# google-research/weatherbenchX

Hardware: AMD Instinct MI355X
Metric: grid-point·metric evals/s (0.25° 721×1440×37L) at 1/2/4/8 GPUs; % HBM roofline (higher is better)
Workload: dtype f32+f64

## Files before the change

include/wbx.h:

```cpp
#ifndef WBX_H_
#define WBX_H_

#include <stddef.h>
#include <stdint.h>

#ifdef __cplusplus
extern "C" {
#endif

#define WBX_ABI_VERSION 13

typedef enum wbx_status {
  WBX_OK = 0,
  WBX_ERR_INVALID = -1,
  WBX_ERR_HIP = -2,
  WBX_ERR_NO_DEVICE = -3,
  WBX_ERR_FFT = -4,
  WBX_ERR_RCCL = -5
} wbx_status;

typedef struct wbx_ctx wbx_ctx;

typedef enum wbx_dtype { WBX_F32 = 0, WBX_F64 = 1 } wbx_dtype;

typedef enum wbx_det_func { WBX_DET3 = 0, WBX_DET6 = 1, WBX_PASS1 = 2 } wbx_det_func;
#define WBX_DET3_LANES 3
#define WBX_DET6_LANES 6
#define WBX_PASS1_LANES 1

#define WBX_ENS_LANES 5
typedef enum wbx_ens_algo {
  WBX_ENS_SORT = 0,
  WBX_ENS_PAIRWISE = 1
} wbx_ens_algo;

#define WBX_FLAG_MASKED 1u
#define WBX_FLAG_SKIPNA 2u
#define WBX_FLAG_FAIR   4u
#define WBX_FLAG_SKIPNA_ENS 8u

#define WBX_MAX_INPUTS 4

typedef struct wbx_s1_plan {
  int64_t nkey;
  int64_t ndepth;
  int64_t nx;
  int32_t x_kept;
  int32_t nchunk;
  int64_t depth_chunk;
  int64_t xstride[WBX_MAX_INPUTS];
  const int64_t* key_off[WBX_MAX_INPUTS];
  const int64_t* depth_off[WBX_MAX_INPUTS];
  const int32_t* gather_key;
  const int32_t* gather_depth;
  const int64_t* gather_tab;
  int32_t n_gather_depth;
  uint32_t flags;
  int32_t block_threads;
  int32_t vec;
  int32_t plane_rows;
  int32_t reserved_;
  const double* x_weights;
} wbx_s1_plan;

int wbx_s1_partial_len(const wbx_s1_plan* plan, int lanes, int64_t* n_out);

int wbx_abi_version(void);
const char* wbx_last_error(void);
int wbx_device_count(int* n_out);
int wbx_ctx_create(int device_id, void* hip_stream, wbx_ctx** out);
int wbx_ctx_destroy(wbx_ctx* ctx);
int wbx_ctx_synchronize(wbx_ctx* ctx);
int wbx_ctx_device_name(wbx_ctx* ctx, char* buf, size_t buflen);

int wbx_malloc(wbx_ctx* ctx, size_t bytes, void** dptr_out);
int wbx_free(wbx_ctx* ctx, void* dptr);
int wbx_memcpy_h2d(wbx_ctx* ctx, void* dptr, const void* h_src, size_t bytes);
int wbx_memcpy_d2h(wbx_ctx* ctx, void* h_dst, const void* dptr, size_t bytes);
int wbx_memset(wbx_ctx* ctx, void* dptr, int value, size_t bytes);

typedef struct wbx_fence wbx_fence;
int wbx_host_alloc(wbx_ctx* ctx, size_t bytes, void** h_out);
int wbx_host_free(wbx_ctx* ctx, void* h_ptr);
int wbx_memcpy_d2h_async(wbx_ctx* ctx, void* h_pinned, const void* dptr, size_t bytes);
int wbx_fence_create(wbx_ctx* ctx, wbx_fence** out);
int wbx_fence_record(wbx_ctx* ctx, wbx_fence* fence);
int wbx_fence_wait(wbx_fence* fence);
int wbx_fence_destroy(wbx_fence* fence);
int wbx_ctx_wait_fence(wbx_ctx* ctx, wbx_fence* fence);
int wbx_memcpy_h2d_async(wbx_ctx* ctx, void* dptr, const void* h_pinned, size_t bytes);
int wbx_memcpy_d2d(wbx_ctx* ctx, void* dst, const void* src, size_t bytes);
int wbx_host_transpose(void* dst, const void* src, int64_t batch, int64_t rows, int64_t cols, int32_t elem_bytes);
int wbx_clock_probe(wbx_ctx* ctx, int32_t blocks, double* shader_mhz_out);

int wbx_acc_add(wbx_ctx* ctx, double* acc, const double* src, int64_t n, int32_t overwrite);

#define WBX_COMM_ID_BYTES 128
typedef struct wbx_comm wbx_comm;
int wbx_comm_unique_id(void* id_out );
int wbx_comm_create(wbx_ctx* ctx, const void* unique_id, int32_t nranks, int32_t rank, wbx_comm** out);
int wbx_comm_destroy(wbx_comm* comm);
int wbx_comm_info(const wbx_comm* comm, int32_t* nranks_out, int32_t* rank_out, int64_t* collectives_out);
int wbx_acc_allreduce(wbx_ctx* ctx, wbx_comm* comm, double* acc, int64_t n);
int wbx_acc_read(wbx_ctx* ctx, const double* acc, int64_t n, double* host_out);
int wbx_acc_reset(wbx_ctx* ctx, double* acc, int64_t n);

int wbx_notnan_mask(wbx_ctx* ctx, const void* data, int dtype, int64_t n, uint8_t* valid_out);

int wbx_timer_start(wbx_ctx* ctx);
int wbx_timer_stop(wbx_ctx* ctx, float* ms_out);
int wbx_mark(wbx_ctx* ctx, int* index_out);
int wbx_mark_elapsed(wbx_ctx* ctx, int i0, int i1, float* ms_out);
int wbx_marks_reset(wbx_ctx* ctx);

int wbx_det_partial(wbx_ctx* ctx, const wbx_s1_plan* plan, int func ,
                    int dtype , const void* p, const void* t, const void* c,
                    const uint8_t* mask, double* partial_out);

int wbx_ens_partial(wbx_ctx* ctx, const wbx_s1_plan* plan, int dtype, int M,
                    int64_t member_stride, int algo , const void* p,
                    const void* t, const uint8_t* mask, double* partial_out);

#define WBX_ENS2_LANES 2
int wbx_ens2_partial(wbx_ctx* ctx, const wbx_s1_plan* plan, int dtype, int M, int64_t member_stride, int N,
                     int64_t target_member_stride, const void* p, const void* t, const uint8_t* mask, double* partial_out);

typedef struct wbx_s2_plan {
  int64_t nA, nBk, nBr, nchunk, nlane, nj, nbin;
  int32_t sum_j;
} wbx_s2_plan;
int wbx_contract(wbx_ctx* ctx, const wbx_s2_plan* plan, const double* partial,
                 const double* W, double* out);

int wbx_contract_bits(wbx_ctx* ctx, const wbx_s2_plan* plan, const double* partial, const double* wt,
                      const uint64_t* bits, double* out);

typedef enum wbx_cat_func { WBX_CAT_EXCEED = 0, WBX_CAT_RANK = 1 } wbx_cat_func;
int wbx_cat_partial(wbx_ctx* ctx, const wbx_s1_plan* plan, int func, int dtype, int ncat, int M,
                    int64_t member_stride, const void* p, const void* t, const double* thresholds,
                    const uint8_t* mask, double* partial_out);
int wbx_cat_exceed_field(wbx_ctx* ctx, const wbx_s1_plan* plan, int dtype, int ncat, int M, int64_t member_stride,
                         const void* p, const void* t, const double* threshold_field, int64_t category_stride,
                         const uint8_t* mask, double* partial_out);

#define WBX_CONT_CELLS 4
#define WBX_CONT_MAX_THRESHOLDS 16
int wbx_contingency_partial(wbx_ctx* ctx, const wbx_s1_plan* plan, int dtype , int nthr,
                            const void* p, const void* t, const double* thresholds ,
                            const uint8_t* mask, double* partial_out);

#define WBX_ERPS_MAX_THRESHOLDS 16
#define WBX_ERPS_MAX_MEMBERS 256
int wbx_ens_rps_partial(wbx_ctx* ctx, const wbx_s1_plan* plan, int dtype , int M, int64_t member_stride,
                        int nthr, const double* p_thresholds, const double* t_thresholds ,
                        int right_inclusive, const void* p, const void* t, const uint8_t* mask, double* partial_out);

#define WBX_ENRG_LANES 2
#define WBX_ENRG_MAX_MEMBERS 64
int wbx_ens_energy_partial(wbx_ctx* ctx, const wbx_s1_plan* plan, int dtype , int M, int64_t member_stride,
                           int64_t L, int64_t p_norm_stride, int64_t t_norm_stride, const void* p, const void* t,
                           const uint8_t* mask, double* partial_out);

#define WBX_BINNED_W_ON_X 1
#define WBX_BINNED_WT_X_ONLY 2
#define WBX_BINNED_WT_ROW_ONLY 4
#define WBX_BINNED_TWIN_MASK 16
#define WBX_BINNED_ACCUMULATE 32
#define WBX_BINNED_MASK_ON_W 8
int wbx_det_binned(wbx_ctx* ctx, const wbx_s1_plan* plan, int func, int dtype, const void* p, const void* t,
                   const void* c, const uint8_t* mask, const double* wt, const uint64_t* bits, int64_t nA,
                   int64_t nBk, int64_t nBr, int32_t w_on_x, int32_t nbin, const void* atoms, double* out);
int wbx_binned_atoms_size(const wbx_s1_plan* plan, int64_t nA, int64_t nBk, int64_t nBr, int32_t w_on_x,
                          int64_t* bytes_out);
int wbx_binned_atoms(wbx_ctx* ctx, const wbx_s1_plan* plan, int64_t nA, int64_t nBk, int64_t nBr, int32_t w_on_x,
                     const uint64_t* bits, void* atoms_out );

int wbx_ens_binned(wbx_ctx* ctx, const wbx_s1_plan* plan, int dtype, int M, int64_t member_stride, int algo, const void* p,
                   const void* t, const uint8_t* mask, const double* wt, const uint64_t* bits, int64_t nA, int64_t nBk,
                   int64_t nBr, int32_t w_on_x, int32_t nbin, const void* atoms, double* out);
int wbx_ens_binned_atoms_size(const wbx_s1_plan* plan, int64_t nA, int64_t nBk, int64_t nBr, int32_t w_on_x,
                              int64_t* bytes_out);
int wbx_ens_binned_atoms(wbx_ctx* ctx, const wbx_s1_plan* plan, int64_t nA, int64_t nBk, int64_t nBr, int32_t w_on_x,
                         const uint64_t* bits, void* atoms_out ,
                         int64_t* overflow_out );

int wbx_det_map(wbx_ctx* ctx, const wbx_s1_plan* plan, int func, int dtype, int lane,
                const void* p, const void* t, const void* c, double* out);
int wbx_ens_map(wbx_ctx* ctx, const wbx_s1_plan* plan, int dtype, int M, int64_t member_stride,
                int algo, int lane, const void* p, const void* t, double* out);

int wbx_zonal_spectrum(wbx_ctx* ctx, const float* field, int64_t lon_stride, int64_t row_stride, int64_t nrows,
                       int32_t nlon, const int32_t* group, const double* scale, int32_t ngroup,
                       int32_t accumulate, double* power_out);

int wbx_zonal_spectrum_slabs(wbx_ctx* ctx, const float* field, int64_t lon_stride, int64_t row_stride,
                             int64_t rows_per_slab, int64_t nslab, const int64_t* h_slab_offsets, int32_t nlon,
                             const int32_t* group, const double* scale, int32_t ngroup, int32_t accumulate,
                             double* power_out);

int wbx_det_spectrum(wbx_ctx* ctx, const wbx_s1_plan* plan, int func , int dtype ,
                     const void* p, const void* t, const void* c, const int32_t* group, const double* scale, int64_t ngroup,
                     double* partial_out, double* power_p, double* power_t);

int wbx_det_spectrum_folded(wbx_ctx* ctx, const wbx_s1_plan* plan, int func , int dtype ,
                            const void* p, const void* t, const void* c, const int32_t* group, const double* scale,
                            const double* det_scale, int64_t ngroup, double* det_out, double* power_p, double* power_t);

int wbx_det_spectrum_slabs(wbx_ctx* ctx, const wbx_s1_plan* plan, int func , int dtype ,
                           const void* p, const void* t, const void* c, int64_t rows_per_slab, const int32_t* group,
                           const double* scale, int64_t ngroup, double* partial_out, double* power_p, double* power_t);

typedef enum wbx_fn {
  WBX_FN_DET_PARTIAL = 1, WBX_FN_ENS_PARTIAL = 2, WBX_FN_ENS2_PARTIAL = 3, WBX_FN_CAT_PARTIAL = 4, WBX_FN_CAT_EXCEED_FIELD = 5,
  WBX_FN_CONTRACT = 6, WBX_FN_CONTRACT_BITS = 7, WBX_FN_DET_BINNED = 8, WBX_FN_ENS_BINNED = 9, WBX_FN_ZONAL_SPECTRUM = 10,
  WBX_FN_ZONAL_SPECTRUM_SLABS = 11, WBX_FN_DET_SPECTRUM = 12, WBX_FN_DET_SPECTRUM_SLABS = 13, WBX_FN_ACC_ADD = 14,
  WBX_FN_MEMSET = 15, WBX_FN_MEMCPY_D2D = 16, WBX_FN_CTX_WAIT_FENCE = 17, WBX_FN_FENCE_RECORD = 18, WBX_FN_DET_SPECTRUM_FOLDED = 19,
  WBX_FN_CONTINGENCY_PARTIAL = 20, WBX_FN_ENS_RPS_PARTIAL = 21, WBX_FN_ENS_ENERGY_PARTIAL = 22
} wbx_fn;
#define WBX_CALL_MAX_ARGS 20
typedef struct wbx_call {
  int32_t fn;
  int32_t nargs;
  uint64_t args[WBX_CALL_MAX_ARGS];
} wbx_call;
typedef struct wbx_reloc {
  int32_t call, arg, slot, reserved_;
  int64_t offset;
} wbx_reloc;
int wbx_chunk_replay(wbx_call* calls, int32_t ncalls, const wbx_reloc* relocs, int32_t nrelocs, const uint64_t* slots,
                     int32_t nslots);

#ifdef __cplusplus
}
#endif
#endif
```

weatherbenchx_amd/_hip.py:

```python
from __future__ import annotations

import ctypes as C
import os
import threading

import numpy as np

_LIB_NAME = 'libwbx_hip.so'
_LIB_PATH = os.environ.get('WBX_LIBRARY_PATH') or os.path.join(os.path.dirname(os.path.abspath(__file__)), _LIB_NAME)

MAX_INPUTS = 4
F32, F64 = 0, 1
DET3, DET6, PASS1 = 0, 1, 2
DET_LANES = {DET3: 3, DET6: 6, PASS1: 1}
DET_INPUTS = {DET3: 2, DET6: 3, PASS1: 1}
CAT_EXCEED, CAT_RANK = 0, 1
CONT_CELLS = 4
CONT_MAX_THRESHOLDS = 16
ERPS_MAX_THRESHOLDS = 16
ERPS_MAX_MEMBERS = 256
ENRG_LANES = 2
ENRG_MAX_MEMBERS = 64
ENRG_LDS_CHUNK = 16
ENS_LANES = 5
ENS2_LANES = 2
ENS_SORT, ENS_PAIRWISE = 0, 1
COMM_ID_BYTES = 128
FLAG_MASKED, FLAG_SKIPNA, FLAG_FAIR, FLAG_SKIPNA_ENS = 1, 2, 4, 8
BINNED_W_ON_X, BINNED_WT_X_ONLY, BINNED_WT_ROW_ONLY, BINNED_MASK_ON_W, BINNED_TWIN_MASK = 1, 2, 4, 8, 16
BINNED_ACCUMULATE = 32

EXPORTED_SYMBOLS = (
    'wbx_abi_version', 'wbx_last_error', 'wbx_device_count', 'wbx_ctx_create', 'wbx_ctx_destroy',
    'wbx_ctx_synchronize', 'wbx_ctx_device_name', 'wbx_malloc', 'wbx_free', 'wbx_memcpy_h2d',
    'wbx_memcpy_d2h', 'wbx_memset', 'wbx_timer_start', 'wbx_timer_stop', 'wbx_mark', 'wbx_mark_elapsed', 'wbx_marks_reset', 'wbx_s1_partial_len',
    'wbx_det_partial', 'wbx_ens_partial', 'wbx_contract', 'wbx_contract_bits', 'wbx_det_binned', 'wbx_cat_partial', 'wbx_det_map', 'wbx_ens_map',
    'wbx_zonal_spectrum', 'wbx_zonal_spectrum_slabs', 'wbx_host_alloc', 'wbx_host_free', 'wbx_memcpy_d2h_async', 'wbx_fence_create',
    'wbx_fence_record', 'wbx_fence_wait', 'wbx_fence_destroy', 'wbx_ctx_wait_fence', 'wbx_memcpy_h2d_async',
    'wbx_memcpy_d2d', 'wbx_acc_add', 'wbx_notnan_mask', 'wbx_binned_atoms_size', 'wbx_binned_atoms',
    'wbx_comm_unique_id', 'wbx_comm_create', 'wbx_comm_destroy', 'wbx_comm_info', 'wbx_acc_allreduce', 'wbx_acc_read',
    'wbx_acc_reset', 'wbx_det_spectrum', 'wbx_det_spectrum_slabs', 'wbx_ens_binned', 'wbx_ens_binned_atoms_size', 'wbx_ens_binned_atoms',
    'wbx_ens2_partial', 'wbx_cat_exceed_field', 'wbx_chunk_replay', 'wbx_host_transpose', 'wbx_clock_probe', 'wbx_det_spectrum_folded',
    'wbx_contingency_partial', 'wbx_ens_rps_partial', 'wbx_ens_energy_partial',
)

FN_IDS = {'wbx_det_partial': 1, 'wbx_ens_partial': 2, 'wbx_ens2_partial': 3, 'wbx_cat_partial': 4, 'wbx_cat_exceed_field': 5,
          'wbx_contract': 6, 'wbx_contract_bits': 7, 'wbx_det_binned': 8, 'wbx_ens_binned': 9, 'wbx_zonal_spectrum': 10,
          'wbx_zonal_spectrum_slabs': 11, 'wbx_det_spectrum': 12, 'wbx_det_spectrum_slabs': 13, 'wbx_acc_add': 14,
          'wbx_memset': 15, 'wbx_memcpy_d2d': 16, 'wbx_ctx_wait_fence': 17, 'wbx_fence_record': 18, 'wbx_det_spectrum_folded': 19,
          'wbx_contingency_partial': 20, 'wbx_ens_rps_partial': 21, 'wbx_ens_energy_partial': 22}
CALL_MAX_ARGS = 20
QUERY_FNS = frozenset({'wbx_s1_partial_len', 'wbx_binned_atoms_size', 'wbx_ens_binned_atoms_size', 'wbx_last_error',
                       'wbx_abi_version', 'wbx_device_count', 'wbx_comm_info'})
HOST_FENCE_FNS = frozenset({'wbx_fence_create', 'wbx_fence_record', 'wbx_fence_wait', 'wbx_fence_destroy'})


def enrg_tile_points(m: int, threads: int) -> int:
  mp = (m + 4) // 4 * 4
  nblk = (mp // 4) * (mp // 4 + 1) // 2
  return max(1, min(64, 416 // mp, 3 * threads // nblk))


class CallStruct(C.Structure):
  _fields_ = [('fn', C.c_int32), ('nargs', C.c_int32), ('args', C.c_uint64 * CALL_MAX_ARGS)]


class RelocStruct(C.Structure):
  _fields_ = [('call', C.c_int32), ('arg', C.c_int32), ('slot', C.c_int32), ('reserved_', C.c_int32), ('offset', C.c_int64)]


RECORDER = None
PROTOS: dict = {}


class _RecordingLib:

  def __init__(self, lib):
    self.__dict__['_lib'] = lib

  def __getattr__(self, name):
    fn = getattr(self._lib, name)
    if name not in PROTOS:
      return fn

    def call(*args, _fn=fn, _name=name):
      rec = RECORDER
      if rec is not None and rec.thread == threading.get_ident():
        rec.note(_name, args)
      return _fn(*args)
    self.__dict__[name] = call
    return call



class WbxUnavailableError(RuntimeError):
  """libwbx_hip.so missing or no MI355X visible -- the product path has no CPU fallback."""


class WbxError(RuntimeError):
  pass


class S1PlanStruct(C.Structure):
  _fields_ = [
      ('nkey', C.c_int64), ('ndepth', C.c_int64), ('nx', C.c_int64),
      ('x_kept', C.c_int32), ('nchunk', C.c_int32), ('depth_chunk', C.c_int64),
      ('xstride', C.c_int64 * MAX_INPUTS),
      ('key_off', C.c_void_p * MAX_INPUTS),
      ('depth_off', C.c_void_p * MAX_INPUTS),
      ('gather_key', C.c_void_p), ('gather_depth', C.c_void_p), ('gather_tab', C.c_void_p),
      ('n_gather_depth', C.c_int32), ('flags', C.c_uint32),
      ('block_threads', C.c_int32), ('vec', C.c_int32), ('plane_rows', C.c_int32), ('reserved_', C.c_int32), ('x_weights', C.c_void_p),
  ]


class S2PlanStruct(C.Structure):
  _fields_ = [(n, C.c_int64) for n in ('nA', 'nBk', 'nBr', 'nchunk', 'nlane', 'nj', 'nbin')] + [('sum_j', C.c_int32)]


_lib = None
_lib_lock = threading.Lock()


def lib_path() -> str:
  return _LIB_PATH


def load_library():
  global _lib
  with _lib_lock:
    if _lib is not None:
      return _lib
    if not os.path.exists(_LIB_PATH):
      raise WbxUnavailableError(
          f'{_LIB_PATH} not found: build it with `python -c "import __graft_entry__ as g; g.build()"` '
          '(make -C weatherbenchx_amd/csrc). There is no CPU fallback.')
    try:
      lib = C.CDLL(_LIB_PATH, mode=C.RTLD_GLOBAL)
    except OSError as e:
      raise WbxUnavailableError(f'cannot load {_LIB_PATH}: {e}') from e
    vp, i32, i64 = C.c_void_p, C.c_int, C.c_int64
    lib.wbx_last_error.restype = C.c_char_p
    lib.wbx_abi_version.restype = i32
    protos = {
        'wbx_device_count': [C.POINTER(i32)],
        'wbx_ctx_create': [i32, vp, C.POINTER(vp)],
        'wbx_ctx_destroy': [vp],
        'wbx_ctx_synchronize': [vp],
        'wbx_ctx_device_name': [vp, C.c_char_p, C.c_size_t],
        'wbx_malloc': [vp, C.c_size_t, C.POINTER(vp)],
        'wbx_free': [vp, vp],
        'wbx_memcpy_h2d': [vp, vp, vp, C.c_size_t],
        'wbx_memcpy_d2h': [vp, vp, vp, C.c_size_t],
        'wbx_memset': [vp, vp, i32, C.c_size_t],
        'wbx_host_alloc': [vp, C.c_size_t, C.POINTER(vp)],
        'wbx_host_free': [vp, vp],
        'wbx_memcpy_d2h_async': [vp, vp, vp, C.c_size_t],
        'wbx_fence_create': [vp, C.POINTER(vp)],
        'wbx_fence_record': [vp, vp],
        'wbx_fence_wait': [vp],
        'wbx_fence_destroy': [vp],
        'wbx_ctx_wait_fence': [vp, vp],
        'wbx_memcpy_h2d_async': [vp, vp, vp, C.c_size_t],
        'wbx_memcpy_d2d': [vp, vp, vp, C.c_size_t],
        'wbx_acc_add': [vp, vp, vp, i64, i32],
        'wbx_notnan_mask': [vp, vp, i32, i64, vp],
        'wbx_comm_unique_id': [vp],
        'wbx_comm_create': [vp, vp, C.c_int32, C.c_int32, C.POINTER(vp)],
        'wbx_comm_destroy': [vp],
        'wbx_comm_info': [vp, C.POINTER(C.c_int32), C.POINTER(C.c_int32), C.POINTER(i64)],
        'wbx_acc_allreduce': [vp, vp, vp, i64],
        'wbx_acc_read': [vp, vp, i64, vp],
        'wbx_acc_reset': [vp, vp, i64],
        'wbx_timer_start': [vp],
        'wbx_timer_stop': [vp, C.POINTER(C.c_float)],
        'wbx_mark': [vp, C.POINTER(i32)],
        'wbx_mark_elapsed': [vp, i32, i32, C.POINTER(C.c_float)],
        'wbx_marks_reset': [vp],
        'wbx_s1_partial_len': [C.POINTER(S1PlanStruct), i32, C.POINTER(i64)],
        'wbx_det_partial': [vp, C.POINTER(S1PlanStruct), i32, i32, vp, vp, vp, vp, vp],
        'wbx_ens_partial': [vp, C.POINTER(S1PlanStruct), i32, i32, i64, i32, vp, vp, vp, vp],
        'wbx_contract': [vp, C.POINTER(S2PlanStruct), vp, vp, vp],
        'wbx_contract_bits': [vp, C.POINTER(S2PlanStruct), vp, vp, vp, vp],
        'wbx_det_binned': [vp, C.POINTER(S1PlanStruct), i32, i32, vp, vp, vp, vp, vp, vp, i64, i64, i64, C.c_int32, C.c_int32, vp, vp],
        'wbx_binned_atoms_size': [C.POINTER(S1PlanStruct), i64, i64, i64, C.c_int32, C.POINTER(i64)],
        'wbx_binned_atoms': [vp, C.POINTER(S1PlanStruct), i64, i64, i64, C.c_int32, vp, vp],
        'wbx_ens_binned': [vp, C.POINTER(S1PlanStruct), i32, i32, i64, i32, vp, vp, vp, vp, vp, i64, i64, i64, C.c_int32, C.c_int32, vp, vp],
        'wbx_ens_binned_atoms_size': [C.POINTER(S1PlanStruct), i64, i64, i64, C.c_int32, C.POINTER(i64)],
        'wbx_ens_binned_atoms': [vp, C.POINTER(S1PlanStruct), i64, i64, i64, C.c_int32, vp, vp, C.POINTER(i64)],
        'wbx_ens2_partial': [vp, C.POINTER(S1PlanStruct), i32, i32, i64, i32, i64, vp, vp, vp, vp],
        'wbx_cat_exceed_field': [vp, C.POINTER(S1PlanStruct), i32, i32, i32, i64, vp, vp, vp, i64, vp, vp],
        'wbx_cat_partial': [vp, C.POINTER(S1PlanStruct), i32, i32, i32, i32, i64, vp, vp, vp, vp, vp],
        'wbx_contingency_partial': [vp, C.POINTER(S1PlanStruct), i32, i32, vp, vp, vp, vp, vp],
        'wbx_ens_rps_partial': [vp, C.POINTER(S1PlanStruct), i32, i32, i64, i32, vp, vp, i32, vp, vp, vp, vp],
        'wbx_ens_energy_partial': [vp, C.POINTER(S1PlanStruct), i32, i32, i64, i64, i64, i64, vp, vp, vp, vp],
        'wbx_det_map': [vp, C.POINTER(S1PlanStruct), i32, i32, i32, vp, vp, vp, vp],
        'wbx_ens_map': [vp, C.POINTER(S1PlanStruct), i32, i32, i64, i32, i32, vp, vp, vp],
        'wbx_zonal_spectrum': [vp, vp, i64, i64, i64, C.c_int32, vp, vp, C.c_int32, C.c_int32, vp],
        'wbx_det_spectrum': [vp, C.POINTER(S1PlanStruct), i32, i32, vp, vp, vp, vp, vp, i64, vp, vp, vp],
        'wbx_det_spectrum_slabs': [vp, C.POINTER(S1PlanStruct), i32, i32, vp, vp, vp, i64, vp, vp, i64, vp, vp, vp],
        'wbx_det_spectrum_folded': [vp, C.POINTER(S1PlanStruct), i32, i32, vp, vp, vp, vp, vp, vp, i64, vp, vp, vp],
        'wbx_zonal_spectrum_slabs': [vp, vp, i64, i64, i64, i64, vp, C.c_int32, vp, vp, C.c_int32, C.c_int32, vp],
    }
    protos['wbx_chunk_replay'] = [vp, i32, vp, i32, vp, i32]
    protos['wbx_host_transpose'] = [vp, vp, i64, i64, i64, C.c_int32]
    protos['wbx_clock_probe'] = [vp, C.c_int32, C.POINTER(C.c_double)]
    for name, argtypes in protos.items():
      fn = getattr(lib, name)
      fn.argtypes = argtypes
      fn.restype = i32
    PROTOS.update(protos)
    _lib = _RecordingLib(lib)
    return _lib


def check(rc: int, what: str = ''):
  if rc != 0:
    msg = load_library().wbx_last_error().decode(errors='replace')
    if rc == -3:
      raise WbxUnavailableError(f'{what}: {msg}')
    raise WbxError(f'{what} failed (status {rc}): {msg}')


def device_count() -> int:
  lib = load_library()
  n = C.c_int(0)
  rc = lib.wbx_device_count(C.byref(n))
  return int(n.value) if rc == 0 else 0


def is_available() -> bool:
  try:
    return device_count() > 0
  except WbxUnavailableError:
    return False


class DeviceBuffer:

  def __init__(self, ctx: 'Context', nbytes: int):
    self.ctx = ctx
    self.nbytes = int(nbytes)
    with ctx._pool_lock:
      free = ctx._dev_free.get(self.nbytes)
      ptr = free.pop() if free else 0
      if ptr:
        ctx._dev_cached -= self.nbytes
    rec = RECORDER
    if rec is not None and rec.thread == threading.get_ident():
      rec.pinned.append(self)
    if not ptr:
      p = C.c_void_p(0)
      rc = ctx.lib.wbx_malloc(ctx.handle, self.nbytes, C.byref(p))
      if rc != 0 and ctx._dev_cached:
        ctx.release_pool()
        rc = ctx.lib.wbx_malloc(ctx.handle, self.nbytes, C.byref(p))
      check(rc, 'wbx_malloc')
      ptr = p.value or 0
    self.ptr = ptr

  def __del__(self):
    try:
      ctx = self.ctx
      if getattr(self, 'ptr', 0) and ctx.handle:
        with ctx._pool_lock:
          if ctx._dev_cached + self.nbytes <= DEVICE_POOL_LIMIT_BYTES:
            ctx._dev_free.setdefault(self.nbytes, []).append(self.ptr)
            ctx._dev_cached += self.nbytes
            self.ptr = 0
        if self.ptr:
          ctx.lib.wbx_free(ctx.handle, C.c_void_p(self.ptr))
          self.ptr = 0
    except Exception:
      pass


DEVICE_POOL_LIMIT_BYTES = int(os.environ.get('WBX_DEVICE_POOL_BYTES', 32 << 30))


class PinnedBlock:

  def __init__(self, ctx: 'Context', ptr: int, capacity: int, nbytes: int, typestr: str = '<f8', itemsize: int = 8):
    self._ctx, self._ptr, self._capacity = ctx, ptr, capacity
    self.__array_interface__ = {'shape': (nbytes // itemsize,), 'typestr': typestr, 'data': (ptr, False), 'version': 3}

  @property
  def ptr(self) -> int:
    return self._ptr

  def __del__(self):
    try:
      self._ctx._pinned_free.setdefault(self._capacity, []).append(self._ptr)
    except Exception:
      pass


def _pinned_block_of(arr):
  base = arr
  while isinstance(base, np.ndarray):
    base = base.base
  return base if isinstance(base, PinnedBlock) else None


def is_pinned(arr) -> bool:
  return _pinned_block_of(arr) is not None


def is_loader_pinned(arr) -> bool:
  block = _pinned_block_of(arr)
  return block is not None and getattr(block, 'for_loader', False)


class Fence:

  def __init__(self, ctx: 'Context'):
    self._lib = ctx.lib
    h = C.c_void_p(0)
    check(ctx.lib.wbx_fence_create(ctx.handle, C.byref(h)), 'wbx_fence_create')
    self._h = h
    check(ctx.lib.wbx_fence_record(ctx.handle, h), 'wbx_fence_record')
    self._done = False

  def wait(self):
    if not self._done:
      check(self._lib.wbx_fence_wait(self._h), 'wbx_fence_wait')
      self._done = True

  def __del__(self):
    try:
      if self._h:
        self.wait()
        self._lib.wbx_fence_destroy(self._h)
        self._h = None
    except Exception:
      pass


ALL_CONTEXTS = None


class Context:

  def __init__(self, device_id: int = 0, stream_ptr: int | None = None):
    global ALL_CONTEXTS
    if ALL_CONTEXTS is None:
      import weakref
      ALL_CONTEXTS = weakref.WeakSet()
    ALL_CONTEXTS.add(self)
    self.lib = load_library()
    h = C.c_void_p(0)
    check(self.lib.wbx_ctx_create(int(device_id), C.c_void_p(stream_ptr or 0), C.byref(h)), 'wbx_ctx_create')
    self.handle = h
    self.device_id = int(device_id)
    self._pinned_free: dict[int, list[int]] = {}
    self._dev_free: dict[int, list[int]] = {}
    self._dev_cached = 0
    self._pool_lock = threading.Lock()

  def release_pool(self):
    with self._pool_lock:
      blocks, self._dev_free, self._dev_cached = self._dev_free, {}, 0
# ... 132 lines not shown
```

weatherbenchx_amd/csrc/wbx_common.hpp:

```cpp
#pragma once
#include <hip/hip_runtime.h>

#include <cstdarg>
#include <cstdint>
#include <cstdio>
#include <cstring>

#include "../../include/wbx.h"

struct wbx_ctx {
  int device = 0;
  int num_cus = 256;
  hipStream_t stream = nullptr;
  bool own_stream = false;
  hipEvent_t ev_start = nullptr;
  hipEvent_t ev_stop = nullptr;
  void* fft_state = nullptr;
  void* s2_scratch = nullptr;
  size_t s2_scratch_size = 0;
  void* aidm_scratch = nullptr;
  size_t aidm_scratch_size = 0;
  void* atoms_clean = nullptr;
  void* patch_counters = nullptr;
  size_t patch_counters_size = 0;
  hipEvent_t* marks = nullptr;
  int marks_used = 0, marks_made = 0, marks_cap = 0;
};

namespace wbx {

char* last_error_buf();

inline int fail(int code, const char* fmt, ...) {
  va_list ap;
  va_start(ap, fmt);
  vsnprintf(last_error_buf(), 512, fmt, ap);
  va_end(ap);
  return code;
}

template <typename T>
__device__ __forceinline__ T ld_stream(const T* p) {
  return __builtin_nontemporal_load(p);
}

__device__ __forceinline__ const char* uniform_ptr(const char* p) {
  const uint64_t v = (uint64_t)p;
  const uint32_t lo = __builtin_amdgcn_readfirstlane((uint32_t)v), hi = __builtin_amdgcn_readfirstlane((uint32_t)(v >> 32));
  return (const char*)(((uint64_t)hi << 32) | lo);
}

template <typename T>
using global_ptr = const __attribute__((address_space(1))) T*;

template <typename T>
using const_ptr = const __attribute__((address_space(4))) T*;

static __constant__ int64_t wbx_zero_i64[1] = {0};
static __constant__ double wbx_one_f64[1] = {1.0};

__device__ __forceinline__ int64_t readlane64(int64_t v, int j) {
  const int lo = __builtin_amdgcn_readlane((int)(uint32_t)(uint64_t)v, j);
  const int hi = __builtin_amdgcn_readlane((int)(uint32_t)((uint64_t)v >> 32), j);
  return (int64_t)(((uint64_t)(uint32_t)hi << 32) | (uint32_t)lo);
}

__device__ __forceinline__ double wave_sum(double v) {
#pragma unroll
  for (int o = 32; o > 0; o >>= 1) v += __shfl_xor(v, o, 64);
  return v;
}

__device__ __forceinline__ int64_t wave_sum_i64(int64_t v) {
#pragma unroll
  for (int o = 32; o > 0; o >>= 1) v += (int64_t)__shfl_xor((long long)v, o, 64);
  return v;
}

template <int CTRL, int ROW_MASK>
__device__ __forceinline__ double dpp_moved(double v) {
  const int lo = __builtin_amdgcn_update_dpp(0, __double2loint(v), CTRL, ROW_MASK, 0xf, true);
  const int hi = __builtin_amdgcn_update_dpp(0, __double2hiint(v), CTRL, ROW_MASK, 0xf, true);
  return __hiloint2double(hi, lo);
}

__device__ __forceinline__ double wave_sum_lane63(double v) {
  v += dpp_moved<0xB1, 0xf>(v);
  v += dpp_moved<0x4E, 0xf>(v);
  v += dpp_moved<0x124, 0xf>(v);
  v += dpp_moved<0x128, 0xf>(v);
  v += dpp_moved<0x142, 0xa>(v);
  v += dpp_moved<0x143, 0xc>(v);
  return v;
}

__device__ __forceinline__ double wave_sum_uniform(double v) {
  const double t = wave_sum_lane63(v);
  return __hiloint2double(__builtin_amdgcn_readlane(__double2hiint(t), 63), __builtin_amdgcn_readlane(__double2loint(t), 63));
}

}

#define WBX_HIP(expr)                                                                   \
  do {                                                                                  \
    hipError_t _e = (expr);                                                             \
    if (_e != hipSuccess)                                                               \
      return wbx::fail(WBX_ERR_HIP, "%s failed: %s (%s:%d)", #expr, hipGetErrorString(_e), \
                       __FILE__, __LINE__);                                             \
  } while (0)

#define WBX_REQUIRE(cond, ...)                                   \
  do {                                                           \
    if (!(cond)) return wbx::fail(WBX_ERR_INVALID, __VA_ARGS__); \
  } while (0)
```

weatherbenchx_amd/csrc/wbx_ctx.hip:

```cpp
#include <cstdlib>

#include <set>

#include "wbx_common.hpp"

namespace wbx {
char* last_error_buf() {
  static thread_local char buf[512] = "";
  return buf;
}
}

extern "C" int wbx_abi_version(void) { return WBX_ABI_VERSION; }

extern "C" const char* wbx_last_error(void) { return wbx::last_error_buf(); }

extern "C" int wbx_device_count(int* n_out) {
  WBX_REQUIRE(n_out != nullptr, "n_out is NULL");
  int n = 0;
  hipError_t e = hipGetDeviceCount(&n);
  if (e != hipSuccess) {
    *n_out = 0;
    return wbx::fail(WBX_ERR_NO_DEVICE, "hipGetDeviceCount: %s", hipGetErrorString(e));
  }
  *n_out = n;
  return 0;
}

extern "C" int wbx_ctx_create(int device_id, void* hip_stream, wbx_ctx** out) {
  WBX_REQUIRE(out != nullptr, "out is NULL");
  *out = nullptr;
  int n = 0;
  if (hipGetDeviceCount(&n) != hipSuccess || n <= 0)
    return wbx::fail(WBX_ERR_NO_DEVICE, "no HIP device visible (libwbx_hip has no CPU path)");
  WBX_REQUIRE(device_id >= 0 && device_id < n, "device_id %d out of range [0,%d)", device_id, n);
  WBX_HIP(hipSetDevice(device_id));
  wbx_ctx* c = new wbx_ctx();
  c->device = device_id;
  int cus = 0;
  if (hipDeviceGetAttribute(&cus, hipDeviceAttributeMultiprocessorCount, device_id) == hipSuccess && cus > 0) c->num_cus = cus;
  if (hip_stream) {
    c->stream = reinterpret_cast<hipStream_t>(hip_stream);
    c->own_stream = false;
  } else {
    hipError_t e = hipStreamCreateWithFlags(&c->stream, hipStreamNonBlocking);
    if (e != hipSuccess) {
      delete c;
      return wbx::fail(WBX_ERR_HIP, "hipStreamCreate: %s", hipGetErrorString(e));
    }
    c->own_stream = true;
  }
  if (hipEventCreate(&c->ev_start) != hipSuccess || hipEventCreate(&c->ev_stop) != hipSuccess) {
    delete c;
    return wbx::fail(WBX_ERR_HIP, "hipEventCreate failed");
  }
  *out = c;
  return 0;
}

namespace wbx {
void spectrum_release(wbx_ctx* ctx);
void spectrum_note_write(const void* dst, size_t bytes);
}

extern "C" int wbx_ctx_destroy(wbx_ctx* ctx) {
  if (!ctx) return 0;
  (void)hipSetDevice(ctx->device);
  (void)hipStreamSynchronize(ctx->stream);
  wbx::spectrum_release(ctx);
  if (ctx->s2_scratch) (void)hipFree(ctx->s2_scratch);
  if (ctx->aidm_scratch) (void)hipFree(ctx->aidm_scratch);
  if (ctx->patch_counters) (void)hipFree(ctx->patch_counters);
  delete static_cast<std::set<const void*>*>(ctx->atoms_clean);
  if (ctx->ev_start) (void)hipEventDestroy(ctx->ev_start);
  if (ctx->ev_stop) (void)hipEventDestroy(ctx->ev_stop);
  for (int i = 0; i < ctx->marks_made; ++i) (void)hipEventDestroy(ctx->marks[i]);
  free(ctx->marks);
  if (ctx->own_stream && ctx->stream) (void)hipStreamDestroy(ctx->stream);
  delete ctx;
  return 0;
}

extern "C" int wbx_ctx_synchronize(wbx_ctx* ctx) {
  WBX_REQUIRE(ctx != nullptr, "ctx is NULL");
  WBX_HIP(hipStreamSynchronize(ctx->stream));
  return 0;
}

extern "C" int wbx_ctx_device_name(wbx_ctx* ctx, char* buf, size_t buflen) {
  WBX_REQUIRE(ctx != nullptr && buf != nullptr && buflen > 0, "bad arguments");
  hipDeviceProp_t prop;
  WBX_HIP(hipGetDeviceProperties(&prop, ctx->device));
  snprintf(buf, buflen, "%s|%s|cus=%d", prop.name, prop.gcnArchName, prop.multiProcessorCount);
  return 0;
}

extern "C" int wbx_malloc(wbx_ctx* ctx, size_t bytes, void** dptr_out) {
  WBX_REQUIRE(ctx != nullptr && dptr_out != nullptr, "bad arguments");
  *dptr_out = nullptr;
  if (bytes == 0) return 0;
  WBX_HIP(hipSetDevice(ctx->device));
  WBX_HIP(hipMalloc(dptr_out, bytes));
  return 0;
}

extern "C" int wbx_free(wbx_ctx* ctx, void* dptr) {
  WBX_REQUIRE(ctx != nullptr, "ctx is NULL");
  if (!dptr) return 0;
  WBX_HIP(hipSetDevice(ctx->device));
  WBX_HIP(hipStreamSynchronize(ctx->stream));
  {
    hipDeviceptr_t base = nullptr;
    size_t size = 0;
    if (hipMemGetAddressRange(&base, &size, dptr) != hipSuccess) {
      (void)hipGetLastError();
      size = 1;
    }
    wbx::spectrum_note_write(dptr, size);
  }
  WBX_HIP(hipFree(dptr));
  return 0;
}

extern "C" int wbx_memcpy_h2d(wbx_ctx* ctx, void* dptr, const void* h_src, size_t bytes) {
  WBX_REQUIRE(ctx != nullptr, "ctx is NULL");
  if (bytes == 0) return 0;
  WBX_REQUIRE(dptr != nullptr && h_src != nullptr, "NULL pointer");
  WBX_HIP(hipSetDevice(ctx->device));
  wbx::spectrum_note_write(dptr, bytes);
  WBX_HIP(hipMemcpyAsync(dptr, h_src, bytes, hipMemcpyHostToDevice, ctx->stream));
  WBX_HIP(hipStreamSynchronize(ctx->stream));
  return 0;
}

extern "C" int wbx_memcpy_d2h(wbx_ctx* ctx, void* h_dst, const void* dptr, size_t bytes) {
  WBX_REQUIRE(ctx != nullptr, "ctx is NULL");
  if (bytes == 0) return 0;
  WBX_REQUIRE(dptr != nullptr && h_dst != nullptr, "NULL pointer");
  WBX_HIP(hipSetDevice(ctx->device));
  WBX_HIP(hipMemcpyAsync(h_dst, dptr, bytes, hipMemcpyDeviceToHost, ctx->stream));
  WBX_HIP(hipStreamSynchronize(ctx->stream));
  return 0;
}

extern "C" int wbx_host_alloc(wbx_ctx* ctx, size_t bytes, void** h_out) {
  WBX_REQUIRE(ctx != nullptr && h_out != nullptr, "NULL argument");
  WBX_HIP(hipSetDevice(ctx->device));
  WBX_HIP(hipHostMalloc(h_out, bytes ? bytes : 8, hipHostMallocDefault));
  return 0;
}

extern "C" int wbx_host_free(wbx_ctx* ctx, void* h_ptr) {
  WBX_REQUIRE(ctx != nullptr, "ctx is NULL");
  if (h_ptr) WBX_HIP(hipHostFree(h_ptr));
  return 0;
}

extern "C" int wbx_memcpy_d2h_async(wbx_ctx* ctx, void* h_pinned, const void* dptr, size_t bytes) {
  WBX_REQUIRE(ctx != nullptr, "ctx is NULL");
  if (bytes == 0) return 0;
  WBX_REQUIRE(dptr != nullptr && h_pinned != nullptr, "NULL pointer");
  WBX_HIP(hipSetDevice(ctx->device));
  WBX_HIP(hipMemcpyAsync(h_pinned, dptr, bytes, hipMemcpyDeviceToHost, ctx->stream));
  return 0;
}

struct wbx_fence {
  hipEvent_t ev;
};

extern "C" int wbx_fence_create(wbx_ctx* ctx, wbx_fence** out) {
  WBX_REQUIRE(ctx != nullptr && out != nullptr, "NULL argument");
  WBX_HIP(hipSetDevice(ctx->device));
  wbx_fence* f = new wbx_fence;
  hipError_t e = hipEventCreateWithFlags(&f->ev, hipEventDisableTiming);
  if (e != hipSuccess) {
    delete f;
    WBX_HIP(e);
  }
  *out = f;
  return 0;
}

extern "C" int wbx_fence_record(wbx_ctx* ctx, wbx_fence* f) {
  WBX_REQUIRE(ctx != nullptr && f != nullptr, "NULL argument");
  WBX_HIP(hipEventRecord(f->ev, ctx->stream));
  return 0;
}

extern "C" int wbx_fence_wait(wbx_fence* f) {
  WBX_REQUIRE(f != nullptr, "fence is NULL");
  WBX_HIP(hipEventSynchronize(f->ev));
  return 0;
}

extern "C" int wbx_ctx_wait_fence(wbx_ctx* ctx, wbx_fence* f) {
  WBX_REQUIRE(ctx != nullptr && f != nullptr, "NULL argument");
  WBX_HIP(hipStreamWaitEvent(ctx->stream, f->ev, 0));
  return 0;
}

extern "C" int wbx_fence_destroy(wbx_fence* f) {
  if (f) {
    (void)hipEventDestroy(f->ev);
    delete f;
  }
  return 0;
}

extern "C" int wbx_memset(wbx_ctx* ctx, void* dptr, int value, size_t bytes) {
  WBX_REQUIRE(ctx != nullptr, "ctx is NULL");
  if (bytes == 0) return 0;
  WBX_REQUIRE(dptr != nullptr, "NULL pointer");
  wbx::spectrum_note_write(dptr, bytes);
  WBX_HIP(hipMemsetAsync(dptr, value, bytes, ctx->stream));
  return 0;
}

extern "C" int wbx_timer_start(wbx_ctx* ctx) {
  WBX_REQUIRE(ctx != nullptr, "ctx is NULL");
  WBX_HIP(hipEventRecord(ctx->ev_start, ctx->stream));
  return 0;
}

extern "C" int wbx_mark(wbx_ctx* ctx, int* index_out) {
// ... 78 lines not shown
```

weatherbenchx_amd/csrc/wbx_ens.hip:

```cpp
#include "wbx_ens_atoms.hpp"
#include "wbx_ens_impl.hpp"

namespace wbx {

static int ens_common(wbx_ctx* ctx, const wbx_s1_plan* plan, int dtype, int M, int64_t member_stride, int algo,
                      const void* p, const void* t, const uint8_t* mask, double* out, bool map, int lane) {
  if (int rc = s1_begin("", ctx, plan)) return rc;
  WBX_REQUIRE(plan->vec == 1, "ensemble kernels use vec=1");
  WBX_REQUIRE(M >= 1, "ensemble size must be >= 1 (got %d)", M);
  WBX_REQUIRE(algo == WBX_ENS_SORT || algo == WBX_ENS_PAIRWISE || (algo == WBX_ENS_DIAG_LOADONLY && (M == 50 || M == 51)) ||
                  (algo == WBX_ENS_DIAG_PAIRWISE_LDS && M == 51),
              "unknown ensemble algorithm %d", algo);
  S1Args a;
  if (int rc = s1_operands({"", "output pointer", "predictions/targets pointer"}, ctx, plan, 2, p, t, mask, out, a)) return rc;
  a.M = M;
  a.mstride = member_stride;
  a.lane = lane;
  if (dtype == WBX_F64) return launch_ens_op<EnsOpGeneric<double>>(ctx, plan, a, map);
  WBX_REQUIRE(dtype == WBX_F32, "unknown dtype %d", dtype);
  if (plan->flags & WBX_FLAG_SKIPNA_ENS) {
    static const bool generic = getenv("WBX_ENS_SKIPNA_GENERIC") && atoi(getenv("WBX_ENS_SKIPNA_GENERIC")) != 0;
    if (generic || M > 64) return launch_ens_op<EnsOpGeneric<float>>(ctx, plan, a, map);
    algo = WBX_ENS_SKIPNA_SORT;
  }
  if (M == 51) return launch_ens_m51(ctx, plan, a, algo, map);
  if (M == 50) return launch_ens_m50(ctx, plan, a, algo, map);
  if (M <= 4) return launch_ens_m4(ctx, plan, a, algo, map);
  if (M <= 8) return launch_ens_m8(ctx, plan, a, algo, map);
  if (M <= 16) return launch_ens_m16(ctx, plan, a, algo, map);
  if (M <= 32) return launch_ens_m32(ctx, plan, a, algo, map);
  if (M <= 64) return launch_ens_m64(ctx, plan, a, algo, map);
  return launch_ens_op<EnsOpGeneric<float>>(ctx, plan, a, map);
}

}

extern "C" int wbx_ens_partial(wbx_ctx* ctx, const wbx_s1_plan* plan, int dtype, int M, int64_t member_stride,
                               int algo, const void* p, const void* t, const uint8_t* mask, double* partial_out) {
  return wbx::ens_common(ctx, plan, dtype, M, member_stride, algo, p, t, mask, partial_out, false, 0);
}

extern "C" int wbx_ens_map(wbx_ctx* ctx, const wbx_s1_plan* plan, int dtype, int M, int64_t member_stride, int algo,
                           int lane, const void* p, const void* t, double* out) {
  if (lane < 0 || lane >= WBX_ENS_LANES) return wbx::fail(WBX_ERR_INVALID, "ensemble lane %d out of range", lane);
  return wbx::ens_common(ctx, plan, dtype, M, member_stride, algo, p, t, nullptr, out, true, lane);
}

namespace wbx {

static int ens_binned_geometry(const wbx_s1_plan* plan, int64_t nA, int64_t nBk, int64_t nBr, int32_t w_on_x, BinnedArgs& g) {
  if (int rc = check_plan(plan)) return rc;
  WBX_REQUIRE(nA >= 1 && nBk >= 1 && nBr >= 1 && plan->nx >= 1 && plan->ndepth >= 1, "empty geometry");
  patch_geometry(g, nA * nBk, nBk, nBr, (w_on_x & WBX_BINNED_W_ON_X) ? plan->nx : 1, plan->ndepth, plan->nx, ENS_ATOMS_ROWS);
  return 0;
}

}

extern "C" int wbx_ens_binned_atoms_size(const wbx_s1_plan* plan, int64_t nA, int64_t nBk, int64_t nBr, int32_t w_on_x,
                                         int64_t* bytes_out) {
  using namespace wbx;
  WBX_REQUIRE(bytes_out != nullptr, "bytes_out is NULL");
  BinnedArgs g;
  if (int rc = ens_binned_geometry(plan, nA, nBk, nBr, w_on_x, g)) return rc;
  *bytes_out = (int64_t)atoms_carve(g, nullptr);
  return 0;
}

extern "C" int wbx_ens_binned_atoms(wbx_ctx* ctx, const wbx_s1_plan* plan, int64_t nA, int64_t nBk, int64_t nBr,
                                    int32_t w_on_x, const uint64_t* bits, void* atoms_out, int64_t* overflow_out) {
  using namespace wbx;
  WBX_REQUIRE(ctx != nullptr, "ctx is NULL");
  WBX_REQUIRE(bits != nullptr && atoms_out != nullptr, "NULL pointer");
  BinnedArgs g;
  if (int rc = ens_binned_geometry(plan, nA, nBk, nBr, w_on_x, g)) return rc;
  WBX_HIP(hipSetDevice(ctx->device));
  atoms_carve(g, atoms_out);
  if (int rc = atoms_launch(ctx, g, bits, plan->ndepth, plan->nx, true)) return rc;
  if (overflow_out) {
    const size_t n = (size_t)g.nBk * g.nrs * g.nxt;
    int32_t* host = (int32_t*)malloc(n * sizeof(int32_t));
    WBX_REQUIRE(host != nullptr, "out of host memory");
    hipError_t err = hipMemcpyAsync(host, g.nwords, n * sizeof(int32_t), hipMemcpyDeviceToHost, ctx->stream);
    if (err == hipSuccess) err = hipStreamSynchronize(ctx->stream);
    int64_t bad = 0;
    for (size_t i = 0; i < n && err == hipSuccess; ++i) bad += host[i] < 0;
    free(host);
    WBX_HIP(err);
    *overflow_out = bad;
  }
  return 0;
}

extern "C" int wbx_ens_binned(wbx_ctx* ctx, const wbx_s1_plan* plan, int dtype, int M, int64_t member_stride, int algo,
                              const void* p, const void* t, const uint8_t* mask, const double* wt, const uint64_t* bits,
                              int64_t nA, int64_t nBk, int64_t nBr, int32_t w_on_x, int32_t nbin, const void* atoms,
                              double* out) {
  using namespace wbx;
  WBX_REQUIRE(ctx != nullptr, "ctx is NULL");
  if (int rc = check_plan(plan)) return rc;
  WBX_REQUIRE(dtype == WBX_F32, "wbx_ens_binned takes float32 members (got dtype %d)", dtype);
  WBX_REQUIRE(algo == WBX_ENS_SORT, "wbx_ens_binned runs the rank form (WBX_ENS_SORT) only");
  WBX_REQUIRE(M >= 2 && M <= 64, "wbx_ens_binned handles 2..64 members (got %d)", M);
  WBX_REQUIRE(!(plan->flags & WBX_FLAG_SKIPNA_ENS), "wbx_ens_binned does not take skipna_ensemble (per-point member counts)");
  WBX_REQUIRE(nbin >= 1 && nbin <= 64, "wbx_ens_binned handles 1..64 bins (got %d)", nbin);
  WBX_REQUIRE(nA >= 0 && nBk >= 0 && nBr >= 0 && nA * nBk * nBr == plan->nkey, "nA*nBk*nBr must equal plan->nkey");
  WBX_REQUIRE((w_on_x & ~63) == 0 && (w_on_x & 6) != 6, "w_on_x: unknown or contradictory WBX_BINNED_* flags (%d)", w_on_x);
  WBX_REQUIRE(wt == nullptr || (w_on_x & (WBX_BINNED_WT_X_ONLY | WBX_BINNED_WT_ROW_ONLY)),
              "wbx_ens_binned takes factored weights only (WBX_BINNED_WT_X_ONLY / WBX_BINNED_WT_ROW_ONLY), or wt = NULL");
  WBX_REQUIRE(!(w_on_x & WBX_BINNED_WT_X_ONLY) || (w_on_x & WBX_BINNED_W_ON_X), "WBX_BINNED_WT_X_ONLY needs WBX_BINNED_W_ON_X");
  const bool twin_out = (plan->flags & WBX_FLAG_MASKED) && (w_on_x & WBX_BINNED_TWIN_MASK);
  const bool skipna = (plan->flags & WBX_FLAG_SKIPNA) != 0;
  const int64_t nout = nA * nBk * (skipna ? (twin_out ? 20 : 10) : (twin_out ? ENS_ATOMS_NOUT2 : ENS_ATOMS_NOUT)) * nbin;
  if (nout == 0) return 0;
  WBX_REQUIRE(out != nullptr, "out is NULL");
  WBX_HIP(hipSetDevice(ctx->device));
  if (nBr * plan->ndepth * plan->nx == 0) {
    if (!(w_on_x & WBX_BINNED_ACCUMULATE)) WBX_HIP(hipMemsetAsync(out, 0, (size_t)nout * sizeof(double), ctx->stream));
    return 0;
  }
  WBX_REQUIRE(p != nullptr && t != nullptr && bits != nullptr, "p/t/bits is NULL");
  if (plan->flags & WBX_FLAG_MASKED) {
    WBX_REQUIRE(mask != nullptr, "WBX_FLAG_MASKED set but mask is NULL");
    WBX_REQUIRE(w_on_x & WBX_BINNED_W_ON_X, "wbx_ens_binned with a validity mask needs W indexed per x (WBX_BINNED_W_ON_X)");
    WBX_REQUIRE(plan->xstride[3] >= 0, "the mask's x stride must be non-negative");
  }
  WBX_REQUIRE(plan->xstride[0] >= 0 && plan->xstride[1] >= 0 && (double)plan->nx * (double)plan->xstride[0] * 4.0 < 4294967296.0 &&
                  (double)plan->nx * (double)plan->xstride[1] * 4.0 < 4294967296.0,
              "x offsets of the members and of the targets must be non-negative and fit 32 bits");
  S1Args a;
  fill_args(plan, a);
  a.in[0] = p;
  a.in[1] = t;
  a.in[3] = mask;
  a.M = M;
  a.mstride = member_stride;
  EnsBinnedCall c;
  c.wt = wt;
  c.bits = bits;
  c.nA = nA;
  c.nBk = nBk;
  c.nBr = nBr;
  c.nj = (w_on_x & WBX_BINNED_W_ON_X) ? plan->nx : 1;
  c.nbin = nbin;
  c.w_on_x = w_on_x;
  c.prepared = atoms;
  c.out = out;
  if (M == 51) return launch_ens_atoms_m51(ctx, plan, a, c);
  if (M == 50) return launch_ens_atoms_m50(ctx, plan, a, c);
  if (M <= 4) return launch_ens_atoms_m4(ctx, plan, a, c);
  if (M <= 8) return launch_ens_atoms_m8(ctx, plan, a, c);
  if (M <= 16) return launch_ens_atoms_m16(ctx, plan, a, c);
  if (M <= 32) return launch_ens_atoms_m32(ctx, plan, a, c);
  return launch_ens_atoms_m64(ctx, plan, a, c);
}
```

weatherbenchx_amd/csrc/wbx_ens_atoms.hpp:

```cpp
#pragma once
#include <type_traits>
#include "wbx_aidm.hpp"
#include "wbx_ens_impl.hpp"
#include "wbx_patch.hpp"

namespace wbx {

constexpr int ENS_ATOMS_NQ = 5;
constexpr int ENS_ATOMS_NOUT = 6;
constexpr int ENS_ATOMS_NOUT2 = 12;
constexpr int ENS_ATOMS_ROWS2 = 2 * ATOM_MAX;

constexpr int64_t ENS_ATOMS_ROWS = 16;


constexpr int ENS_ATOMS_G1 = 4;
constexpr int ENS_ATOMS_G2 = 16;

template <typename T>
__device__ __forceinline__ void st_dev(T* p, T v) {
  __hip_atomic_store(p, v, __ATOMIC_RELAXED, __HIP_MEMORY_SCOPE_AGENT);
}
template <typename T>
__device__ __forceinline__ T ld_dev(const T* p) {
  return __hip_atomic_load(p, __ATOMIC_RELAXED, __HIP_MEMORY_SCOPE_AGENT);
}

__device__ __forceinline__ void wave_lds_order() {
  __builtin_amdgcn_fence(__ATOMIC_RELEASE, "wavefront");
  __builtin_amdgcn_wave_barrier();
  __builtin_amdgcn_fence(__ATOMIC_ACQUIRE, "wavefront");
}

__device__ __forceinline__ double ld_sc1(__amdgpu_buffer_rsrc_t rs, uint32_t byte_offset) {
  typedef unsigned int u2 __attribute__((ext_vector_type(2)));
  const u2 v = __builtin_amdgcn_raw_buffer_load_b64(rs, (int)byte_offset, 0, 1 << 4);
  return __hiloint2double((int)v.y, (int)v.x);
}

struct EnsAtomsArgs {
  const double* wx;
  const double* wrow;
  double* tab;
  double* part1;
  double* part2;
  uint32_t* counters;
  uint32_t* unused0;
  int32_t unused1;
  uint32_t* unused2;
  double* out;
  int32_t ng1, ng2;
  int32_t masked;
  int32_t twin_rows;
  int32_t out_mode;
  int32_t accumulate;
  int64_t id_cell_rows;
  int64_t br_per_split;
  unsigned long long* unused3;
};

constexpr int ENS_ATOMS_ROW_BARRIER = 4;

#pragma clang diagnostic push
#pragma clang diagnostic ignored "-Winline-asm"
constexpr int ENS_ATOMS_RAGGED_WPB = 4;
template <int MP, bool EXACT, bool NT, int MODE>
__device__ __forceinline__ void ens_atoms_patch(const S1Args& a, const BinnedArgs& g, const EnsAtomsArgs& e, uint32_t vb,
                                                unsigned char* const lds_raw) {
  constexpr bool SKIPNA = MODE == 2;
  constexpr int WPB = NT ? 1 : ENS_ATOMS_RAGGED_WPB;
  using Op = EnsOpF32<MP, EXACT, WBX_ENS_SORT>;
  constexpr int NQ = ENS_ATOMS_NQ, NOUT = ENS_ATOMS_NOUT;
  constexpr int NLDS = MP < ENS_PIPE_NLDS ? MP : ENS_PIPE_NLDS;
  constexpr int NREG = MP - NLDS;
  constexpr int NONE = 255;
  float(*stage)[64] = reinterpret_cast<float(*)[64]>(lds_raw);
  const int lane = threadIdx.x & 63;
  const int M = EXACT ? MP : a.M;
  int64_t cell;
  int xt, rs;
  if (!patch_decode<WPB>(g, cell, xt, rs, vb)) return;
  const int64_t bk = cell % g.nBk;
  const int64_t A = cell / g.nBk;
  const int64_t npatch = (int64_t)g.nrs * g.nxt;
  const int64_t patch = (int64_t)rs * g.nxt + xt;
  const int nw = g.nwords[bk * npatch + patch];
  constexpr int TR = ENS_ATOMS_ROWS2;
  const bool twin = SKIPNA || e.twin_rows != 0;
  double* const tab = e.tab + (cell * npatch + patch) * (TR * NQ);
  int64_t rbeg, rend;
  int br_first = 0;
  if (g.taper) {
    const const_ptr<int32_t> tab = (const_ptr<int32_t>)g.split_tab;
    br_first = tab[rs];
    rbeg = (int64_t)br_first * a.D;
    rend = (int64_t)tab[rs + 1] * a.D;
  } else {
    const int64_t R = g.nBr * a.D;
    rbeg = (int64_t)rs * g.rows_per_split;
    rend = rbeg + g.rows_per_split < R ? rbeg + g.rows_per_split : R;
  }

  const bool live = (int64_t)xt * 64 + lane < a.nx;
  const uint32_t x = live ? (uint32_t)xt * 64u + (uint32_t)lane : (uint32_t)a.nx - 1u;
  const uint32_t xw = g.nj > 1 ? x : 0u;
  const double w_lane = e.wx ? e.wx[bk * g.nj + xw] : 1.0;
  const uint8_t* const ids = e.masked ? g.aidm : g.aid;
  const uint32_t lds0 = (uint32_t)(uintptr_t)(__attribute__((address_space(3))) void*)&stage[0][0];
  const int64_t mstride_b = a.mstride * 4;
  const unsigned long long live_mask = __builtin_amdgcn_ballot_w64(live);

  int c0 = NONE, c1 = NONE;
  double acc0[NQ], acc1[NQ];
#pragma unroll
  for (int l = 0; l < NQ; ++l) acc0[l] = acc1[l] = 0.0;
  unsigned long long touched = 0ull;
  if (lane < NQ)
    for (int k = 0; k < nw; ++k) {
      st_dev(tab + k * NQ + lane, 0.0);
      if (twin) st_dev(tab + (ATOM_MAX + k) * NQ + lane, 0.0);
    }

  auto flush_all = [&]() {
#pragma unroll 1
    for (int s = 0; s < 2; ++s) {
      const int id = s ? c1 : c0;
      const bool go = id != NONE;
      unsigned long long todo = __builtin_amdgcn_ballot_w64(go);
      while (todo) {
        const int gid = __builtin_amdgcn_readlane(id, __builtin_ctzll(todo));
        const bool sel = go && id == gid;
        double mine = 0.0;
#pragma unroll
        for (int l = 0; l < NQ; ++l) {
          const double sum = wave_sum_uniform(sel ? (s ? acc1[l] : acc0[l]) : 0.0);
          if (lane == l) mine = sum;
        }
        const int row = (gid & (ATOM_MAX - 1)) + ((gid >> 7) ? ATOM_MAX : 0);
        if (lane < NQ) {
          double* q = tab + row * NQ + lane;
          st_dev(q, ((touched >> row) & 1ull) ? ld_dev(q) + mine : mine);
        }
        touched |= 1ull << row;
        todo &= ~__builtin_amdgcn_ballot_w64(sel);
      }
    }
#pragma unroll
    for (int l = 0; l < NQ; ++l) acc0[l] = acc1[l] = 0.0;
    c0 = c1 = NONE;
  };

  const int nrows = nw < 0 ? 0 : (int)(rend - rbeg);
  const int nD = (int)a.D;
  int br_a = g.taper ? br_first : (int)((int64_t)rs * e.br_per_split);
  int d_a = 0;
  const int br_last = (int)((rend - 1) / a.D);
  const int64_t key0 = (A * g.nBk + bk) * g.nBr, wrow0 = bk * g.nBr;
  const bool point_ids = MODE == 1 || (MODE == 2 && e.id_cell_rows != 0);
  const int64_t idrow0 = point_ids ? cell * e.id_cell_rows : wrow0;
  int r_a = (int)rbeg;
  const int r_last = (int)(rend - 1);
  int64_t ra0k = 0, ra0d = 0, ra1k = 0, ra1d = 0, wra = 0;
  double wwa = 1.0;
  const const_ptr<int64_t> zero = (const_ptr<int64_t>)wbx_zero_i64;
  const const_ptr<int64_t> tk0 = a.key_off[0] ? (const_ptr<int64_t>)a.key_off[0] : zero, td0 = a.depth_off[0] ? (const_ptr<int64_t>)a.depth_off[0] : zero;
  const const_ptr<int64_t> tk1 = a.key_off[1] ? (const_ptr<int64_t>)a.key_off[1] : zero, td1 = a.depth_off[1] ? (const_ptr<int64_t>)a.depth_off[1] : zero;
  const const_ptr<double> twr = e.wrow ? (const_ptr<double>)e.wrow : (const_ptr<double>)wbx_one_f64;
  const int64_t mk0 = a.key_off[0] ? -1 : 0, md0 = a.depth_off[0] ? -1 : 0, mk1 = a.key_off[1] ? -1 : 0, md1 = a.depth_off[1] ? -1 : 0,
                mwr = e.wrow ? -1 : 0;
  auto resolve_ahead = [&]() {
    const int64_t key = key0 + br_a;
    ra0k = tk0[key & mk0];
    ra0d = td0[(int64_t)d_a & md0];
    ra1k = tk1[key & mk1];
    ra1d = td1[(int64_t)d_a & md1];
    if constexpr (MODE == 0) {
      wra = (wrow0 + br_a) * g.nj;
    } else {
      wra = (idrow0 + (int64_t)__builtin_amdgcn_readfirstlane(point_ids ? r_a : br_a)) * g.nj;
      r_a = r_a < r_last ? r_a + 1 : r_a;
    }
    wwa = twr[(wrow0 + br_a) & mwr];
    const bool wrap = d_a + 1 == nD;
    d_a = wrap ? 0 : d_a + 1;
    br_a = (wrap && br_a < br_last) ? br_a + 1 : br_a;
  };

  float xn[NREG > 0 ? NREG : 1], tn = 0.f;
  int idn = NONE;
  int64_t ron0 = 0, ron1 = 0;
// ... 368 lines not shown
```

weatherbenchx_amd/csrc/wbx_ens_impl.hpp:

```cpp
#pragma once
#include <cmath>
#include <cstdlib>

#include "wbx_s1.hpp"
#include "wbx_sortnet3_gen.hpp"

namespace wbx {

constexpr int ENS_MIN_WAVES = 1;

constexpr int WBX_ENS_DIAG_LOADONLY = 99;
constexpr int WBX_ENS_DIAG_PAIRWISE_LDS = 98;
constexpr int WBX_ENS_SKIPNA_SORT = 97;

template <typename T>
struct EnsOpGeneric {
  static constexpr int NIN = 2;
  static constexpr int NLANE = WBX_ENS_LANES;
  static constexpr int NACC = WBX_ENS_LANES;
  static constexpr int XR_UNROLL = 1, XK_UNROLL = 1, MIN_WAVES = 1;

  __device__ __forceinline__ static void values(const S1Args& a, const int64_t (&ro)[WBX_MAX_INPUTS], int64_t x,
                                                double (&val)[NLANE]) {
    const int M = a.M;
    const T* pp = reinterpret_cast<const T*>(a.in[0]) + ro[0] + x * a.xstride[0];
    const double td = (double)(reinterpret_cast<const T*>(a.in[1])[ro[1] + x * a.xstride[1]]);
    const bool skip = a.flags & WBX_FLAG_SKIPNA_ENS;
    double se = 0.0, sq = 0.0, sabs = 0.0, pair_total = 0.0, x0 = 0.0;
    int n = 0;
    for (int i = 0; i < M; ++i) {
      const double xi = (double)pp[(int64_t)i * a.mstride];
      if (skip && xi != xi) continue;
      if (n == 0) x0 = xi;
      ++n;
      const double e = xi - x0;
      se += e;
      sq = fma(e, e, sq);
      sabs += fabs(xi - td);
      double row = 0.0;
      for (int j = 0; j < i; ++j) {
        const double xj = (double)pp[(int64_t)j * a.mstride];
        if (skip && xj != xj) continue;
        row += fabs(xi - xj);
      }
      pair_total += row;
    }
    const double dM = (double)n;
    const double fair = (a.flags & WBX_FLAG_FAIR) ? 1.0 : 0.0;
    const double mean_e = se / dM;
    const double mean_d = (x0 - td) + mean_e;
    const double var = (sq - se * mean_e) / (dM - 1.0);
    val[0] = sabs / dM;
    val[1] = 2.0 * pair_total / (dM * (dM - fair));
    val[2] = var;
    val[3] = mean_d * mean_d - var / dM;
    val[4] = mean_d * mean_d;
  }

  template <int V, bool XK>
  __device__ __forceinline__ static void accum(const S1Args& a, const int64_t (&ro)[WBX_MAX_INPUTS], int64_t x,
                                               double (&acc)[XK ? V : 1][NACC]) {
    static_assert(V == 1, "ensemble op is one point per lane");
    double val[NLANE];
    values(a, ro, x, val);
#pragma unroll
    for (int l = 0; l < NLANE; ++l) acc[0][l] += val[l];
  }
};

template <int MP, bool EXACT, int ALGO>
struct EnsOpF32 {
  static constexpr int NIN = 2;
  static constexpr int NLANE = WBX_ENS_LANES;
  static constexpr int NACC = WBX_ENS_LANES;
  static constexpr int XR_UNROLL = 1, XK_UNROLL = 1, MIN_WAVES = ENS_MIN_WAVES;

  struct Regs {
    float xm[MP];
    float t;
    float poison;
  };

  __device__ __forceinline__ static void load(const S1Args& a, const int64_t (&ro)[WBX_MAX_INPUTS], int64_t x, Regs& r) {
    const int M = EXACT ? MP : a.M;
    const float* pp = reinterpret_cast<const float*>(a.in[0]) + ro[0] + x * a.xstride[0];
    r.t = ld_stream(reinterpret_cast<const float*>(a.in[1]) + ro[1] + x * a.xstride[1]);
#pragma unroll
    for (int m = 0; m < MP; ++m) r.xm[m] = (EXACT || m < M) ? ld_stream(pp + (int64_t)m * a.mstride) : INFINITY;
  }

  __device__ __forceinline__ static void values(const S1Args& a, const int64_t (&ro)[WBX_MAX_INPUTS], int64_t x,
                                                double (&val)[NLANE]) {
    Regs r;
    load(a, ro, x, r);
    finish(a, ro, x, r, val);
  }

  template <bool FAST32 = false>
  __device__ __forceinline__ static bool compute(const S1Args& a, Regs& r, double (&val)[NLANE]) {
    const int M = EXACT ? MP : a.M;
    const double td = (double)r.t;
    float(&xm)[MP] = r.xm;

    if constexpr (ALGO == WBX_ENS_DIAG_LOADONLY) {
      float s = 0.f;
#pragma unroll
      for (int m = 0; m < MP; ++m)
        if (EXACT || m < M) s += xm[m];
      val[0] = (double)s - td;
      val[1] = val[2] = val[3] = val[4] = 0.0;
      return false;
    }
    double pair_total = 0.0;
    float poison = 0.f;
    int nvalid = 0;
    bool weird = false;
    float shift32 = 0.f;
    if constexpr (ALGO == WBX_ENS_SKIPNA_SORT) {
      const bool tfin32 = (r.t - r.t) == 0.f;
      shift32 = r.t;
      if (__builtin_amdgcn_ballot_w64(!tfin32)) {
        float lo = INFINITY;
#pragma unroll
        for (int m = 0; m < MP; ++m)
          if (EXACT || m < M) lo = fminf(lo, xm[m]);
        shift32 = tfin32 ? r.t : lo;
      }
#pragma unroll
      for (int m = 0; m < MP; ++m) {
        if (EXACT || m < M) {
          const float x = xm[m];
          const bool missing = x != x;
          nvalid += missing ? 0 : 1;
          xm[m] = missing ? shift32 : x;
        }
      }
      if constexpr (!EXACT) {
        float big = 0.f;
        int m = 0;
        for (; m + 1 < MP; m += 2) {
          const float a = m < M ? xm[m] : 0.f, b = m + 1 < M ? xm[m + 1] : 0.f;
          asm("v_max3_f32 %0, %1, |%2|, |%3|" : "=v"(big) : "v"(big), "v"(a), "v"(b));
        }
        if (m < MP) {
          const float a = m < M ? xm[m] : 0.f;
          asm("v_max3_f32 %0, %1, |%2|, |%2|" : "=v"(big) : "v"(big), "v"(a));
        }
        weird = big == INFINITY;
      }
    }
    if constexpr (ALGO == WBX_ENS_PAIRWISE) {
#pragma unroll
      for (int i = 1; i < MP; ++i) {
        if (EXACT || i < M) {
// ... 141 lines not shown
        if constexpr (ALGO == WBX_ENS_SORT) dot = fma((double)(2 * (m + 1) - M - 1), e, dot);
      }
    }
    sabs += fabs(x0t);
    const double dM = (double)M;
    const double fair = (a.flags & WBX_FLAG_FAIR) ? 1.0 : 0.0;
    const double inv_m = 1.0 / dM, inv_m1 = M > 1 ? 1.0 / (dM - 1.0) : __builtin_nan(""), spread_scale = 2.0 / (dM * (dM - fair));
    const double mean_e = se * inv_m;
    const double mean_d = x0t + mean_e;
    const double var = (sq - se * mean_e) * inv_m1;
    double spread;
    if constexpr (ALGO == WBX_ENS_SORT) {
      spread = dot * spread_scale;
    } else {
      spread = pair_total * spread_scale;
    }
    if constexpr (ALGO == WBX_ENS_DIAG_PAIRWISE_LDS) {
      static_assert(EXACT && MP % 17 == 0, "the LDS-tiled diagnostic is instantiated for M = 51");
      constexpr int B = 17, NB = MP / B;
      __shared__ float tile[MP][64];
      float* col = &tile[0][threadIdx.x];
#pragma unroll
      for (int m = 0; m < MP; ++m) col[m * 64] = xm[m];
      asm volatile("" ::: "memory");
      double total = 0.0;
#pragma unroll
      for (int bi = 0; bi < NB; ++bi) {
        float xi[B];
#pragma unroll
        for (int k = 0; k < B; ++k) xi[k] = col[(bi * B + k) * 64];
#pragma unroll
        for (int k = 1; k < B; ++k) {
          float row = 0.f;
#pragma unroll
          for (int l = 0; l < k; ++l) row += fabsf(xi[k] - xi[l]);
          total += (double)row;
        }
#pragma unroll
        for (int bj = 0; bj < bi; ++bj) {
          float xj[B];
#pragma unroll
          for (int l = 0; l < B; ++l) xj[l] = col[(bj * B + l) * 64];
#pragma unroll
          for (int k = 0; k < B; ++k) {
            float row = 0.f;
#pragma unroll
            for (int l = 0; l < B; ++l) row += fabsf(xi[k] - xj[l]);
            total += (double)row;
          }
        }
      }
      spread = total * spread_scale;
    }
    val[0] = sabs * inv_m;
    val[1] = spread;
    val[2] = var;
    val[3] = mean_d * mean_d - var * inv_m;
    val[4] = mean_d * mean_d;
  }

  __device__ __forceinline__ static void stats32(const S1Args& a, float (&xm)[MP], const float t, const float poison,
                                                 double (&val)[NLANE]) {
    static_assert(EXACT, "fp32 chain sums are instantiated for the exact-M buckets");
    constexpr int K = 8, MID = MP / 2, NPAIR = MP / 2;
    const float c = xm[MID];
    float se[K], sq[K], sa[K], dt[K];
#pragma unroll
    for (int k = 0; k < K; ++k) se[k] = sq[k] = sa[k] = dt[k] = k == 0 ? poison : 0.f;
#pragma unroll
    for (int i = 0; i < NPAIR; ++i) {
      const int j = MP - 1 - i, k = i % K;
      const float ei = xm[i] - c, ej = xm[j] - c;
      se[k] += ei + ej;
      sq[k] = fmaf(ei, ei, sq[k]);
      sq[k] = fmaf(ej, ej, sq[k]);
      sa[k] += fabsf(xm[i] - t);
      sa[k] += fabsf(xm[j] - t);
      dt[k] = fmaf((float)(MP - 1 - 2 * i), xm[j] - xm[i], dt[k]);
    }
    if constexpr (MP & 1) {
      sa[NPAIR % K] += fabsf(c - t);
    } else {
    }
    auto fold = [](const float (&v)[K]) {
      return ((double)(v[0] + v[4]) + (double)(v[1] + v[5])) + ((double)(v[2] + v[6]) + (double)(v[3] + v[7]));
    };
    const double dse = fold(se), dsq = fold(sq), dsa = fold(sa), ddt = fold(dt);
    constexpr double dM = (double)MP;
    const double fair = (a.flags & WBX_FLAG_FAIR) ? 1.0 : 0.0;
    constexpr double inv_m = 1.0 / dM, inv_m1 = 1.0 / (dM - 1.0);
    const double spread_scale = 2.0 / (dM * (dM - fair));
    const double mean_e = dse * inv_m;
    const double mean_d = ((double)c - (double)t) + mean_e;
    const double var = (dsq - dse * mean_e) * inv_m1;
    val[0] = dsa * inv_m;
    val[1] = ddt * spread_scale;
    val[2] = var;
    val[3] = mean_d * mean_d - var * inv_m;
    val[4] = mean_d * mean_d;
  }

  template <int V, bool XK>
  __device__ __forceinline__ static void accum(const S1Args& a, const int64_t (&ro)[WBX_MAX_INPUTS], int64_t x,
                                               double (&acc)[XK ? V : 1][NACC]) {
    static_assert(V == 1, "ensemble op is one point per lane");
    double val[NLANE];
    values(a, ro, x, val);
#pragma unroll
    for (int l = 0; l < NLANE; ++l) acc[0][l] += val[l];
  }
};

template <class Core, bool SKIPNA>
struct EnsMasked {
  static constexpr int NIN = Core::NIN;
  static constexpr int NLANE = Core::NLANE;
  static constexpr int NACC = Core::NLANE + (SKIPNA ? Core::NLANE : 1);
  static constexpr int XR_UNROLL = 1, XK_UNROLL = 1, MIN_WAVES = ENS_MIN_WAVES;

  __device__ __forceinline__ static void values(const S1Args& a, const int64_t (&ro)[WBX_MAX_INPUTS], int64_t x,
                                                double (&val)[NLANE]) {
    Core::values(a, ro, x, val);
  }

  template <int V, bool XK>
  __device__ __forceinline__ static void accum(const S1Args& a, const int64_t (&ro)[WBX_MAX_INPUTS], int64_t x,
                                               double (&acc)[XK ? V : 1][NACC]) {
    static_assert(V == 1, "ensemble op is one point per lane");
    double val[NLANE];
    Core::values(a, ro, x, val);
    const bool valid =
        (a.flags & WBX_FLAG_MASKED) ? reinterpret_cast<const uint8_t*>(a.in[3])[ro[3] + x * a.xstride[3]] != 0 : true;
    if constexpr (!SKIPNA) {
#pragma unroll
      for (int l = 0; l < NLANE; ++l) acc[0][l] += valid ? val[l] : 0.0;
      acc[0][NLANE] += valid ? 1.0 : 0.0;
    } else {
#pragma unroll
      for (int l = 0; l < NLANE; ++l) {
        const bool ok = valid && !(val[l] != val[l]);
        acc[0][l] += ok ? val[l] : 0.0;
        acc[0][NLANE + l] += ok ? 1.0 : 0.0;
      }
    }
  }
};


#pragma clang diagnostic push
#pragma clang diagnostic ignored "-Winline-asm"
constexpr int ENS_PIPE_NLDS = 50;
constexpr int ENS_PIPE_WAVES = 3;
constexpr int ENS_PIPE_SKIPNA_WAVES = 3;
template <int MP, bool EXACT, int ALGO, bool FLAT>
__global__ void __launch_bounds__(64, ALGO == WBX_ENS_SKIPNA_SORT ? ENS_PIPE_SKIPNA_WAVES : ENS_PIPE_WAVES)
ens_pipe_kernel(S1Args a, int R) {
  using Op = EnsOpF32<MP, EXACT, ALGO>;
  constexpr int NA = Op::NACC;
  constexpr int NLDS = MP < ENS_PIPE_NLDS ? MP : ENS_PIPE_NLDS;
  constexpr int NREG = MP - NLDS;
  __shared__ float stage[NLDS][64];
  const int lane = threadIdx.x;
  const int M = EXACT ? MP : a.M;
  const int64_t b = blockIdx.x;
  const int64_t key = b / a.nchunk;
  const int chunk = (int)(b - key * a.nchunk);
  const int64_t d0 = (int64_t)chunk * a.dchunk;
  const int64_t d1 = d0 + a.dchunk < a.D ? d0 + a.dchunk : a.D;
  const int nx = (int)a.nx;
  const uint32_t lds0 = (uint32_t)(uintptr_t)(__attribute__((address_space(3))) void*)&stage[0][0];
  const int64_t mstride_b = a.mstride * 4;

  int64_t kb[WBX_MAX_INPUTS], ro[WBX_MAX_INPUTS];
  key_bases<2>(a, key, kb);
  double acc[NA];
#pragma unroll
  for (int l = 0; l < NA; ++l) acc[l] = 0.0;

  int64_t d = d0, e0 = 0, e1 = 0, et = 0;
  int wm = 0;
  const int wstep = 64 % nx;
  auto open_segment = [&]() {
    if constexpr (FLAT) {
      const int64_t plane = d / R;
      const int64_t j0 = d - plane * R;
      const int64_t nj = d1 - d < R - j0 ? d1 - d : R - j0;
      row_bases<2>(a, kb, key, plane * R, ro);
      e0 = j0 * nx;
      e1 = (j0 + nj) * nx;
      et = e0 & ~(int64_t)63;
      wm = (int)((et + lane) % nx);
      d += nj;
    } else {
      row_bases<2>(a, kb, key, d, ro);
      e0 = 0;
      e1 = nx;
      et = 0;
      d += 1;
    }
  };

  float xn[NREG > 0 ? NREG : 1], tn = 0.f;
  double wn = 0.0;
  auto issue = [&]() {
    int64_t e = et + lane;
    e = e < e0 ? e0 : (e < e1 ? e : e1 - 1);
    const uint32_t voff = (uint32_t)e * (uint32_t)a.xstride[0] * 4u;
    const char* um = uniform_ptr(reinterpret_cast<const char*>(a.in[0]) + ro[0] * 4);
#pragma unroll
    for (int m = 0; m < NLDS; ++m) {
      if (EXACT || m < M)
        asm volatile("s_add_u32 m0, %2, %3\n\tglobal_load_lds_dword %0, %1 nt" ::"v"(voff), "s"(um), "s"(lds0), "i"(m * 256)
                     : "memory", "scc", "m0");
      um += mstride_b;
      asm volatile("" : "+s"(um));
    }
    const float* pr = reinterpret_cast<const float*>(a.in[0]) + ro[0] + e * a.xstride[0];
#pragma unroll
    for (int m = NLDS; m < MP; ++m) xn[m - NLDS] = (EXACT || m < M) ? ld_stream(pr + (int64_t)m * a.mstride) : INFINITY;
    tn = ld_stream(reinterpret_cast<const float*>(a.in[1]) + ro[1] + e * a.xstride[1]);
    if constexpr (FLAT) wn = a.xw[wm];
  };

  bool more = d < d1;
  if (more) {
    open_segment();
    issue();
  }
  while (more) {
    typename Op::Regs r;
    asm volatile("s_waitcnt vmcnt(0)" ::: "memory");
#pragma unroll
    for (int m = 0; m < NLDS; ++m) r.xm[m] = (EXACT || m < M) ? stage[m][lane] : INFINITY;
#pragma unroll
    for (int m = NLDS; m < MP; ++m) r.xm[m] = xn[m - NLDS];
    r.t = tn;
    const double wcur = wn;
    const int64_t ecur = et + lane;
    const bool valid = ecur >= e0 && ecur < e1;
    const int64_t xcur = ecur < e0 ? e0 : (ecur < e1 ? ecur : e1 - 1);
    int64_t rocur[WBX_MAX_INPUTS];
#pragma unroll
    for (int i = 0; i < WBX_MAX_INPUTS; ++i) rocur[i] = ro[i];
    const bool full = et >= e0 && et + 64 <= e1;
    et += 64;
    if (et >= e1) {
      more = d < d1;
      if (more) open_segment();
    } else if constexpr (FLAT) {
      wm += wstep;
      wm = wm >= nx ? wm - nx : wm;
    }
    asm volatile("s_waitcnt lgkmcnt(0)" ::: "memory");
    if (more) issue();
    double val[Op::NLANE];
    Op::template finish<true>(a, rocur, xcur, r, val);
    if constexpr (FLAT) {
      if (full) {
#pragma unroll
        for (int l = 0; l < NA; ++l) acc[l] = fma(val[l], wcur, acc[l]);
      } else {
#pragma unroll
        for (int l = 0; l < NA; ++l) acc[l] = fma(valid ? val[l] : 0.0, wcur, acc[l]);
      }
    } else if (full) {
#pragma unroll
      for (int l = 0; l < NA; ++l) acc[l] += val[l];
    } else {
#pragma unroll
      for (int l = 0; l < NA; ++l) acc[l] += valid ? val[l] : 0.0;
    }
  }
#pragma unroll
  for (int l = 0; l < NA; ++l) {
    const double v = wave_sum(acc[l]);
    if (lane == l) a.out[(key * a.nchunk + chunk) * NA + l] = v;
  }
}

#pragma clang diagnostic pop

inline bool ens_pipe_ok(const wbx_s1_plan* plan, const S1Args& a, bool skipna_ens = false) {
  static const bool off = getenv("WBX_ENS_PIPE") && atoi(getenv("WBX_ENS_PIPE")) == 0;
  static const bool off_skipna = getenv("WBX_ENS_PIPE_SKIPNA") && atoi(getenv("WBX_ENS_PIPE_SKIPNA")) == 0;
  if (off || (skipna_ens && off_skipna)) return false;
  if (plan->x_kept || plan->x_weights != nullptr || plan->block_threads != 64) return false;
  if (plan->flags & (WBX_FLAG_MASKED | WBX_FLAG_SKIPNA | (skipna_ens ? 0u : (unsigned)WBX_FLAG_SKIPNA_ENS))) return false;
  if (plan->nx <= 0 || plan->ndepth <= 0 || plan->nkey <= 0) return false;
  if (a.xstride[0] < 0 || a.xstride[1] < 0) return false;
  return (double)plan->nx * (double)a.xstride[0] * 4.0 < 4294967296.0;
}

inline bool ens_pipe_flat_ok(const wbx_s1_plan* plan, const S1Args& a) {
  static const bool off = getenv("WBX_ENS_PIPE") && atoi(getenv("WBX_ENS_PIPE")) == 0;
  if (off) return false;
  if (plan->x_kept || plan->x_weights == nullptr || plan->block_threads != 64 || plan->plane_rows <= 0) return false;
  if (plan->flags & (WBX_FLAG_MASKED | WBX_FLAG_SKIPNA | WBX_FLAG_SKIPNA_ENS)) return false;
  if (plan->nx <= 0 || plan->nx > WBX_XW_MAX || plan->ndepth <= 0 || plan->nkey <= 0 || plan->ndepth % plan->plane_rows != 0) return false;
  if (a.xstride[0] != 1 || a.xstride[1] != 1) return false;
  return (double)plan->nx * (double)plan->plane_rows * 4.0 < 4294967296.0;
}

template <int MP, bool EXACT, int ALGO, bool FLAT = false>
int launch_ens_pipe(wbx_ctx* ctx, const wbx_s1_plan* plan, S1Args& a) {
  const int64_t grid = plan->nkey * plan->nchunk;
  WBX_REQUIRE(grid < (int64_t)1 << 31, "grid too large (%lld blocks)", (long long)grid);
  hipLaunchKernelGGL((ens_pipe_kernel<MP, EXACT, ALGO, FLAT>), dim3((unsigned)grid), dim3(64), 0, ctx->stream, a,
                     FLAT ? plan->plane_rows : 0);
  WBX_HIP(hipGetLastError());
  return 0;
}

template <class Op>
int launch_ens_op(wbx_ctx* ctx, const wbx_s1_plan* plan, S1Args& a, bool map) {
  if (map) return launch_map<Op>(ctx, plan, a);
  if (plan->x_weights != nullptr) {
    WBX_REQUIRE(!(plan->flags & WBX_FLAG_SKIPNA_ENS), "flat x-weighted mode does not take skipna_ensemble");
    if (plan->flags & WBX_FLAG_SKIPNA) return launch_flat_weighted1<EnsMasked<Op, true>>(ctx, plan, a);
    if (plan->flags & WBX_FLAG_MASKED) return launch_flat_weighted1<EnsMasked<Op, false>>(ctx, plan, a);
    return launch_flat_weighted1<Op>(ctx, plan, a);
  }
  if (plan->flags & WBX_FLAG_SKIPNA) return launch_partial<EnsMasked<Op, true>, 1>(ctx, plan, a);
  if (plan->flags & WBX_FLAG_MASKED) return launch_partial<EnsMasked<Op, false>, 1>(ctx, plan, a);
  return launch_partial<Op, 1>(ctx, plan, a);
}

template <int MP, bool EXACT>
int launch_ens_bucket(wbx_ctx* ctx, const wbx_s1_plan* plan, S1Args& a, int algo, bool map) {
  if (!map && algo == WBX_ENS_SORT && ens_pipe_ok(plan, a)) return launch_ens_pipe<MP, EXACT, WBX_ENS_SORT>(ctx, plan, a);
  if (!map && algo == WBX_ENS_SORT && ens_pipe_flat_ok(plan, a)) return launch_ens_pipe<MP, EXACT, WBX_ENS_SORT, true>(ctx, plan, a);
  if (algo == WBX_ENS_SORT) return launch_ens_op<EnsOpF32<MP, EXACT, WBX_ENS_SORT>>(ctx, plan, a, map);
  if (algo == WBX_ENS_DIAG_LOADONLY) {
    if (!EXACT || map) return fail(WBX_ERR_INVALID, "the load-only diagnostic exists for the exact-M partial kernels only");
    return launch_partial<EnsOpF32<MP, EXACT, WBX_ENS_DIAG_LOADONLY>, 1>(ctx, plan, a);
  }
  if (algo == WBX_ENS_DIAG_PAIRWISE_LDS) {
    if constexpr (EXACT && MP == 51) {
      if (map || plan->x_weights != nullptr || (plan->flags & (WBX_FLAG_MASKED | WBX_FLAG_SKIPNA)) || plan->block_threads != 64)
        return fail(WBX_ERR_INVALID, "the LDS-tiled pair-form diagnostic exists for the plain partial kernels with one-wave blocks only");
      return launch_partial<EnsOpF32<MP, EXACT, WBX_ENS_DIAG_PAIRWISE_LDS>, 1>(ctx, plan, a);
    } else {
      return fail(WBX_ERR_INVALID, "the LDS-tiled pair-form diagnostic exists for M = 51 only");
    }
  }
  if (!map && algo == WBX_ENS_SKIPNA_SORT && ens_pipe_ok(plan, a, true)) return launch_ens_pipe<MP, EXACT, WBX_ENS_SKIPNA_SORT>(ctx, plan, a);
  if (algo == WBX_ENS_SKIPNA_SORT) return launch_ens_op<EnsOpF32<MP, EXACT, WBX_ENS_SKIPNA_SORT>>(ctx, plan, a, map);
  return launch_ens_op<EnsOpF32<MP, EXACT, WBX_ENS_PAIRWISE>>(ctx, plan, a, map);
}

int launch_ens_m4(wbx_ctx*, const wbx_s1_plan*, S1Args&, int, bool);
int launch_ens_m8(wbx_ctx*, const wbx_s1_plan*, S1Args&, int, bool);
int launch_ens_m16(wbx_ctx*, const wbx_s1_plan*, S1Args&, int, bool);
int launch_ens_m32(wbx_ctx*, const wbx_s1_plan*, S1Args&, int, bool);
int launch_ens_m64(wbx_ctx*, const wbx_s1_plan*, S1Args&, int, bool);
int launch_ens_m50(wbx_ctx*, const wbx_s1_plan*, S1Args&, int, bool);
int launch_ens_m51(wbx_ctx*, const wbx_s1_plan*, S1Args&, int, bool);

}
```

weatherbenchx_amd/csrc/wbx_ens_m16.hip:

```cpp
#include "wbx_ens_atoms.hpp"
#include "wbx_ens_impl.hpp"
namespace wbx {
int launch_ens_m16(wbx_ctx* ctx, const wbx_s1_plan* plan, S1Args& a, int algo, bool map) {
  return launch_ens_bucket<16, false>(ctx, plan, a, algo, map);
}
int launch_ens_atoms_m16(wbx_ctx* ctx, const wbx_s1_plan* plan, S1Args& a, const EnsBinnedCall& c) {
  return launch_ens_atoms<16, false>(ctx, plan, a, c);
}
}
```

weatherbenchx_amd/csrc/wbx_ens_m32.hip:

```cpp
#include "wbx_ens_atoms.hpp"
#include "wbx_ens_impl.hpp"
namespace wbx {
int launch_ens_m32(wbx_ctx* ctx, const wbx_s1_plan* plan, S1Args& a, int algo, bool map) {
  return launch_ens_bucket<32, false>(ctx, plan, a, algo, map);
}
int launch_ens_atoms_m32(wbx_ctx* ctx, const wbx_s1_plan* plan, S1Args& a, const EnsBinnedCall& c) {
  return launch_ens_atoms<32, false>(ctx, plan, a, c);
}
}
```

weatherbenchx_amd/csrc/wbx_ens_m4.hip:

```cpp
#include "wbx_ens_atoms.hpp"
#include "wbx_ens_impl.hpp"
namespace wbx {
int launch_ens_m4(wbx_ctx* ctx, const wbx_s1_plan* plan, S1Args& a, int algo, bool map) {
  return launch_ens_bucket<4, false>(ctx, plan, a, algo, map);
}
int launch_ens_atoms_m4(wbx_ctx* ctx, const wbx_s1_plan* plan, S1Args& a, const EnsBinnedCall& c) {
  return launch_ens_atoms<4, false>(ctx, plan, a, c);
}
}
```

weatherbenchx_amd/csrc/wbx_ens_m50.hip:

```cpp
#include "wbx_ens_atoms.hpp"
#include "wbx_ens_impl.hpp"
namespace wbx {
int launch_ens_m50(wbx_ctx* ctx, const wbx_s1_plan* plan, S1Args& a, int algo, bool map) {
  return launch_ens_bucket<50, true>(ctx, plan, a, algo, map);
}
int launch_ens_atoms_m50(wbx_ctx* ctx, const wbx_s1_plan* plan, S1Args& a, const EnsBinnedCall& c) {
  return launch_ens_atoms<50, true>(ctx, plan, a, c);
}
}
```

weatherbenchx_amd/csrc/wbx_ens_m51.hip:

```cpp
#include "wbx_ens_atoms.hpp"
#include "wbx_ens_impl.hpp"
namespace wbx {
int launch_ens_m51(wbx_ctx* ctx, const wbx_s1_plan* plan, S1Args& a, int algo, bool map) {
  return launch_ens_bucket<51, true>(ctx, plan, a, algo, map);
}
int launch_ens_atoms_m51(wbx_ctx* ctx, const wbx_s1_plan* plan, S1Args& a, const EnsBinnedCall& c) {
  return launch_ens_atoms<51, true>(ctx, plan, a, c);
}
}
```

weatherbenchx_amd/csrc/wbx_ens_m64.hip:

```cpp
#include "wbx_ens_atoms.hpp"
#include "wbx_ens_impl.hpp"
namespace wbx {
int launch_ens_m64(wbx_ctx* ctx, const wbx_s1_plan* plan, S1Args& a, int algo, bool map) {
  return launch_ens_bucket<64, false>(ctx, plan, a, algo, map);
}
int launch_ens_atoms_m64(wbx_ctx* ctx, const wbx_s1_plan* plan, S1Args& a, const EnsBinnedCall& c) {
  return launch_ens_atoms<64, false>(ctx, plan, a, c);
}
}
```

weatherbenchx_amd/csrc/wbx_ens_m8.hip:

```cpp
#include "wbx_ens_atoms.hpp"
#include "wbx_ens_impl.hpp"
namespace wbx {
int launch_ens_m8(wbx_ctx* ctx, const wbx_s1_plan* plan, S1Args& a, int algo, bool map) {
  return launch_ens_bucket<8, false>(ctx, plan, a, algo, map);
}
int launch_ens_atoms_m8(wbx_ctx* ctx, const wbx_s1_plan* plan, S1Args& a, const EnsBinnedCall& c) {
  return launch_ens_atoms<8, false>(ctx, plan, a, c);
}
}
```

weatherbenchx_amd/csrc/wbx_replay.hip:

```cpp
#include <type_traits>
#include <utility>

#include "wbx_common.hpp"

namespace wbx {

template <typename T>
static inline T replay_arg(uint64_t v) {
  if constexpr (std::is_pointer_v<T>)
    return reinterpret_cast<T>(static_cast<uintptr_t>(v));
  else
    return static_cast<T>(static_cast<int64_t>(v));
}

template <typename... A, size_t... I>
static inline int replay_invoke(int (*fn)(A...), const uint64_t* a, std::index_sequence<I...>) {
  return fn(replay_arg<A>(a[I])...);
}

template <typename... A>
static inline int replay_call(int (*fn)(A...), const wbx_call& c, const char* name) {
  static_assert(sizeof...(A) <= WBX_CALL_MAX_ARGS, "WBX_CALL_MAX_ARGS too small");
  WBX_REQUIRE(c.nargs == (int32_t)sizeof...(A), "wbx_chunk_replay: %s takes %d arguments, the record holds %d", name, (int)sizeof...(A),
              (int)c.nargs);
  return replay_invoke(fn, c.args, std::index_sequence_for<A...>{});
}

}

extern "C" int wbx_chunk_replay(wbx_call* calls, int32_t ncalls, const wbx_reloc* relocs, int32_t nrelocs, const uint64_t* slots,
                                int32_t nslots) {
  using namespace wbx;
  WBX_REQUIRE(ncalls >= 0 && nrelocs >= 0 && nslots >= 0, "negative count");
  WBX_REQUIRE(ncalls == 0 || calls != nullptr, "calls is NULL");
  WBX_REQUIRE(nrelocs == 0 || (relocs != nullptr && slots != nullptr), "relocs / slots is NULL");
  for (int32_t j = 0; j < nrelocs; ++j) {
    const wbx_reloc& r = relocs[j];
    WBX_REQUIRE(r.call >= 0 && r.call < ncalls && r.slot >= 0 && r.slot < nslots && r.arg >= 0 && r.arg < calls[r.call].nargs &&
                    r.arg < WBX_CALL_MAX_ARGS,
                "wbx_chunk_replay: relocation %d out of range (call %d, arg %d, slot %d)", (int)j, (int)r.call, (int)r.arg, (int)r.slot);
    calls[r.call].args[r.arg] = slots[r.slot] + (uint64_t)r.offset;
  }
#define WBX_REPLAY_CASE(ID, FN) \
  case ID:                      \
    rc = replay_call(FN, c, #FN); \
    break;
  for (int32_t i = 0; i < ncalls; ++i) {
    const wbx_call& c = calls[i];
    int rc = 0;
    switch (c.fn) {
      WBX_REPLAY_CASE(WBX_FN_DET_PARTIAL, wbx_det_partial)
      WBX_REPLAY_CASE(WBX_FN_ENS_PARTIAL, wbx_ens_partial)
      WBX_REPLAY_CASE(WBX_FN_ENS2_PARTIAL, wbx_ens2_partial)
      WBX_REPLAY_CASE(WBX_FN_CAT_PARTIAL, wbx_cat_partial)
      WBX_REPLAY_CASE(WBX_FN_CAT_EXCEED_FIELD, wbx_cat_exceed_field)
      WBX_REPLAY_CASE(WBX_FN_CONTINGENCY_PARTIAL, wbx_contingency_partial)
      WBX_REPLAY_CASE(WBX_FN_ENS_RPS_PARTIAL, wbx_ens_rps_partial)
      WBX_REPLAY_CASE(WBX_FN_ENS_ENERGY_PARTIAL, wbx_ens_energy_partial)
      WBX_REPLAY_CASE(WBX_FN_CONTRACT, wbx_contract)
      WBX_REPLAY_CASE(WBX_FN_CONTRACT_BITS, wbx_contract_bits)
      WBX_REPLAY_CASE(WBX_FN_DET_BINNED, wbx_det_binned)
      WBX_REPLAY_CASE(WBX_FN_ENS_BINNED, wbx_ens_binned)
      WBX_REPLAY_CASE(WBX_FN_ZONAL_SPECTRUM, wbx_zonal_spectrum)
      WBX_REPLAY_CASE(WBX_FN_ZONAL_SPECTRUM_SLABS, wbx_zonal_spectrum_slabs)
      WBX_REPLAY_CASE(WBX_FN_DET_SPECTRUM, wbx_det_spectrum)
      WBX_REPLAY_CASE(WBX_FN_DET_SPECTRUM_SLABS, wbx_det_spectrum_slabs)
      WBX_REPLAY_CASE(WBX_FN_DET_SPECTRUM_FOLDED, wbx_det_spectrum_folded)
      WBX_REPLAY_CASE(WBX_FN_ACC_ADD, wbx_acc_add)
      WBX_REPLAY_CASE(WBX_FN_MEMSET, wbx_memset)
      WBX_REPLAY_CASE(WBX_FN_MEMCPY_D2D, wbx_memcpy_d2d)
      WBX_REPLAY_CASE(WBX_FN_CTX_WAIT_FENCE, wbx_ctx_wait_fence)
      WBX_REPLAY_CASE(WBX_FN_FENCE_RECORD, wbx_fence_record)
      default:
        WBX_REQUIRE(false, "wbx_chunk_replay: call %d names entry point %d, which cannot be part of a record", (int)i, (int)c.fn);
    }
    if (rc != 0) return rc;
  }
#undef WBX_REPLAY_CASE
  return 0;
}
```

weatherbenchx_amd/csrc/wbx_s2.hip:

```cpp
#include "wbx_s1.hpp"

namespace wbx {

constexpr int BG = 8;

__global__ void __launch_bounds__(256) s2_reduce_kernel(wbx_s2_plan p, int fixed_j, int nsplit,
                                                        const double* __restrict__ partial,
                                                        const double* __restrict__ W, double* __restrict__ out) {
  int64_t b = blockIdx.x;
  const int split = (int)(b % nsplit);
  b /= nsplit;
  int64_t jf = 0;
  if (fixed_j) {
    jf = b % p.nj;
    b /= p.nj;
  }
  const int64_t lane = b % p.nlane;
  b /= p.nlane;
  const int64_t bk = b % p.nBk;
  const int64_t A = b / p.nBk;
  const int64_t njc = fixed_j ? 1 : p.nj;
  const int64_t ncj = p.nchunk * njc;
  const int64_t ncontr = p.nBr * ncj;
  const int tl = threadIdx.x & 63, wv = threadIdx.x >> 6;
  __shared__ double red[4][BG];
  const double* pbase = partial + (A * p.nBk + bk) * p.nBr * p.nchunk * p.nlane * p.nj;
  const double* wbase = W + bk * p.nBr * p.nj * p.nbin;
  for (int64_t b0 = 0; b0 < p.nbin; b0 += BG) {
    double acc[BG];
#pragma unroll
    for (int g = 0; g < BG; ++g) acc[g] = 0.0;
    if (!fixed_j && p.nj >= 64) {
      const int64_t nrc = p.nBr * p.nchunk, per = (nrc + nsplit - 1) / nsplit;
      const int64_t rc0 = split * per, rc1 = rc0 + per < nrc ? rc0 + per : nrc;
      int64_t br = rc0 / p.nchunk, ch = rc0 - br * p.nchunk;
      for (int64_t rc = rc0; rc < rc1; ++rc) {
        const double* wrow = wbase + br * p.nj * p.nbin + b0;
        const double* prow = pbase + (rc * p.nlane + lane) * p.nj;
        for (int64_t j = threadIdx.x; j < p.nj; j += blockDim.x) {
          const double v = prow[j];
          const double* w = wrow + j * p.nbin;
#pragma unroll
          for (int g = 0; g < BG; ++g)
            if (b0 + g < p.nbin) acc[g] += v * w[g];
        }
        if (++ch == p.nchunk) {
          ch = 0;
          ++br;
        }
      }
    } else {
      for (int64_t c = threadIdx.x; c < ncontr; c += blockDim.x) {
        const int64_t br = c / ncj;
        const int64_t r = c - br * ncj;
        const int64_t ch = r / njc;
        const int64_t j = fixed_j ? jf : r - ch * njc;
        const double v = pbase[((br * p.nchunk + ch) * p.nlane + lane) * p.nj + j];
        const double* w = wbase + (br * p.nj + j) * p.nbin + b0;
#pragma unroll
        for (int g = 0; g < BG; ++g)
          if (b0 + g < p.nbin) acc[g] += v * w[g];
      }
    }
#pragma unroll
    for (int g = 0; g < BG; ++g) {
      double s = wave_sum(acc[g]);
      if (tl == 0) red[wv][g] = s;
    }
    __syncthreads();
    if (threadIdx.x < BG && b0 + threadIdx.x < p.nbin) {
      double s = 0.0;
      for (int w2 = 0; w2 < (int)(blockDim.x >> 6); ++w2) s += red[w2][threadIdx.x];
      const int64_t o = fixed_j ? (((A * p.nBk + bk) * p.nlane + lane) * p.nj + jf) : ((A * p.nBk + bk) * p.nlane + lane);
      out[(o * nsplit + split) * p.nbin + b0 + threadIdx.x] = s;
    }
    __syncthreads();
  }
}

__global__ void __launch_bounds__(256) s2_keepj_kernel(wbx_s2_plan p, int njtile, const double* __restrict__ partial,
                                                       const double* __restrict__ W, double* __restrict__ out) {
  int64_t b = blockIdx.x;
  const int64_t jt = b % njtile;
  b /= njtile;
  const int64_t lane = b % p.nlane;
  b /= p.nlane;
  const int64_t bk = b % p.nBk;
  const int64_t A = b / p.nBk;
  const int64_t j = jt * blockDim.x + threadIdx.x;
  if (j >= p.nj) return;
  const double* pbase = partial + (A * p.nBk + bk) * p.nBr * p.nchunk * p.nlane * p.nj;
  const double* wbase = W + bk * p.nBr * p.nj * p.nbin;
  double* obase = out + ((((A * p.nBk + bk) * p.nlane + lane) * p.nj) + j) * p.nbin;
  for (int64_t b0 = 0; b0 < p.nbin; b0 += BG) {
    double acc[BG];
#pragma unroll
    for (int g = 0; g < BG; ++g) acc[g] = 0.0;
    for (int64_t br = 0; br < p.nBr; ++br) {
      const double* w = wbase + (br * p.nj + j) * p.nbin + b0;
      for (int64_t ch = 0; ch < p.nchunk; ++ch) {
        const double v = pbase[((br * p.nchunk + ch) * p.nlane + lane) * p.nj + j];
#pragma unroll
        for (int g = 0; g < BG; ++g)
          if (b0 + g < p.nbin) acc[g] += v * w[g];
      }
    }
#pragma unroll
    for (int g = 0; g < BG; ++g)
      if (b0 + g < p.nbin) obase[b0 + g] = acc[g];
  }
}

template <int NB>
__global__ void __launch_bounds__(256) s2_bits_kernel(wbx_s2_plan p, int rows_per_block, int nsplit,
                                                      const double* __restrict__ partial,
                                                      const double* __restrict__ wt,
                                                      const unsigned long long* __restrict__ bits,
                                                      double* __restrict__ out) {
  int64_t b = blockIdx.x;
  const int split = (int)(b % nsplit);
  b /= nsplit;
  const int64_t lane = b % p.nlane;
  b /= p.nlane;
  const int64_t bk = b % p.nBk;
  const int64_t A = b / p.nBk;
  const double* pbase = partial + (A * p.nBk + bk) * p.nBr * p.nchunk * p.nlane * p.nj;
  const double* wbase = wt + bk * p.nBr * p.nj;
  const unsigned long long* bbase = bits + bk * p.nBr * p.nj;
  double acc[NB];
#pragma unroll
  for (int g = 0; g < NB; ++g) acc[g] = 0.0;
  double poison = 0.0;
  const int64_t r0 = p.sum_j ? (int64_t)split * rows_per_block : 0;
  const int64_t r1 = p.sum_j ? (r0 + rows_per_block < p.nBr ? r0 + rows_per_block : p.nBr) : p.nBr;
  const int64_t j0 = p.sum_j ? threadIdx.x : (int64_t)split * blockDim.x + threadIdx.x;
  const int64_t jstep = p.sum_j ? blockDim.x : p.nj;
  for (int64_t br = r0; br < r1; ++br) {
    for (int64_t j = j0; j < p.nj; j += jstep) {
      double v = 0.0;
      for (int64_t ch = 0; ch < p.nchunk; ++ch) v += pbase[((br * p.nchunk + ch) * p.nlane + lane) * p.nj + j];
      const double m = v * wbase[br * p.nj + j];
      poison = fma(m, 0.0, poison);
      const unsigned long long bw = bbase[br * p.nj + j];
      const int lo = (int)(unsigned)bw, hi = (int)(unsigned)(bw >> 32);
      const long long mb = __double_as_longlong(m);
#pragma unroll
      for (int g = 0; g < NB; ++g) {
        const int word = g < 32 ? lo : hi;
        const long long sel = (long long)((word << (31 - (g & 31))) >> 31);
        acc[g] += __longlong_as_double(mb & sel);
      }
    }
  }
  if (!p.sum_j) {
    if (j0 < p.nj) {
      double* o = out + ((((A * p.nBk + bk) * p.nlane + lane) * p.nj) + j0) * p.nbin;
      for (int g = 0; g < NB && g < p.nbin; ++g) o[g] = acc[g] + poison;
    }
    return;
  }
  __shared__ double red[4][NB];
  const int tl = threadIdx.x & 63, wv = threadIdx.x >> 6;
#pragma unroll
  for (int g = 0; g < NB; ++g) {
    const double s = wave_sum(acc[g] + poison);
    if (tl == 0) red[wv][g] = s;
  }
  __syncthreads();
  if (threadIdx.x < NB && threadIdx.x < p.nbin) {
    double s = 0.0;
    for (int w2 = 0; w2 < (int)(blockDim.x >> 6); ++w2) s += red[w2][threadIdx.x];
    out[(((A * p.nBk + bk) * p.nlane + lane) * nsplit + split) * p.nbin + threadIdx.x] = s;
  }
}

__global__ void __launch_bounds__(256) s2_bits_finish_kernel(int64_t nrow, int nsplit, int nbin,
                                                             const double* __restrict__ tmp, double* __restrict__ out) {
  const int64_t i = (int64_t)blockIdx.x * blockDim.x + threadIdx.x;
  if (i >= nrow * nbin) return;
  const int64_t row = i / nbin;
  const int bin = (int)(i - row * nbin);
  double s = 0.0;
  for (int k = 0; k < nsplit; ++k) s += tmp[(row * nsplit + k) * nbin + bin];
  out[i] = s;
}

bool s2_patch_eligible(const wbx_s2_plan& p);
int s2_patch(wbx_ctx* ctx, const wbx_s2_plan& p, const double* partial, const double* wt, const uint64_t* bits,
             double* out);

}

extern "C" int wbx_contract_bits(wbx_ctx* ctx, const wbx_s2_plan* plan, const double* partial, const double* wt,
                                 const uint64_t* bits, double* out) {
  using namespace wbx;
  WBX_REQUIRE(ctx != nullptr && plan != nullptr, "ctx/plan is NULL");
  const wbx_s2_plan& p = *plan;
  WBX_REQUIRE(p.nA >= 0 && p.nBk >= 0 && p.nBr >= 0 && p.nchunk >= 0 && p.nlane >= 0 && p.nj >= 0, "negative extent");
  WBX_REQUIRE(p.nbin >= 1 && p.nbin <= 64, "wbx_contract_bits handles 1..64 bins (got %lld)", (long long)p.nbin);
  const int64_t nrow = p.nA * p.nBk * p.nlane;
  const int64_t nout = nrow * (p.sum_j ? 1 : p.nj) * p.nbin;
  if (nout == 0) return 0;
  WBX_REQUIRE(out != nullptr, "out is NULL");
  WBX_HIP(hipSetDevice(ctx->device));
  if (p.nBr * p.nchunk * (p.sum_j ? p.nj : 1) == 0) {
    WBX_HIP(hipMemsetAsync(out, 0, (size_t)nout * sizeof(double), ctx->stream));
    return 0;
  }
  WBX_REQUIRE(partial != nullptr && wt != nullptr && bits != nullptr, "partial/wt/bits is NULL");
  if (s2_patch_eligible(p)) return s2_patch(ctx, p, partial, wt, bits, out);
  const unsigned long long* b64 = reinterpret_cast<const unsigned long long*>(bits);
  int rows_per_block = 1, nsplit = 1;
  double* dst = out;
  if (p.sum_j) {
    int64_t want = (4096 + nrow - 1) / nrow;
    if (want > p.nBr) want = p.nBr;
    if (want < 1) want = 1;
    rows_per_block = (int)((p.nBr + want - 1) / want);
    nsplit = (int)((p.nBr + rows_per_block - 1) / rows_per_block);
    const size_t need = (size_t)nrow * nsplit * p.nbin * sizeof(double);
    if (ctx->s2_scratch_size < need) {
      if (ctx->s2_scratch) {
        WBX_HIP(hipStreamSynchronize(ctx->stream));
        WBX_HIP(hipFree(ctx->s2_scratch));
      }
      WBX_HIP(hipMalloc(&ctx->s2_scratch, need));
      ctx->s2_scratch_size = need;
    }
    dst = reinterpret_cast<double*>(ctx->s2_scratch);
  } else {
    nsplit = (int)((p.nj + 255) / 256);
  }
  const int64_t grid = nrow * nsplit;
  WBX_REQUIRE(grid < (int64_t)1 << 31, "stage-2 grid too large");
  if (p.nbin <= 16)
    hipLaunchKernelGGL((s2_bits_kernel<16>), dim3((unsigned)grid), dim3(256), 0, ctx->stream, p, rows_per_block, nsplit,
                       partial, wt, b64, dst);
  else if (p.nbin <= 32)
    hipLaunchKernelGGL((s2_bits_kernel<32>), dim3((unsigned)grid), dim3(256), 0, ctx->stream, p, rows_per_block, nsplit,
                       partial, wt, b64, dst);
  else
    hipLaunchKernelGGL((s2_bits_kernel<64>), dim3((unsigned)grid), dim3(256), 0, ctx->stream, p, rows_per_block, nsplit,
                       partial, wt, b64, dst);
  WBX_HIP(hipGetLastError());
  if (p.sum_j) {
    const int64_t n = nrow * p.nbin;
    hipLaunchKernelGGL(s2_bits_finish_kernel, dim3((unsigned)((n + 255) / 256)), dim3(256), 0, ctx->stream, nrow, nsplit,
                       (int)p.nbin, dst, out);
    WBX_HIP(hipGetLastError());
  }
  return 0;
}

extern "C" int wbx_contract(wbx_ctx* ctx, const wbx_s2_plan* plan, const double* partial, const double* W,
                            double* out) {
  WBX_REQUIRE(ctx != nullptr && plan != nullptr, "ctx/plan is NULL");
  const wbx_s2_plan& p = *plan;
  WBX_REQUIRE(p.nA >= 0 && p.nBk >= 0 && p.nBr >= 0 && p.nchunk >= 0 && p.nlane >= 0 && p.nj >= 0 && p.nbin >= 0,
              "negative extent in stage-2 plan");
  const int64_t nout = p.nA * p.nBk * p.nlane * (p.sum_j ? 1 : p.nj) * p.nbin;
  if (nout == 0) return 0;
  WBX_REQUIRE(out != nullptr, "out is NULL");
  WBX_HIP(hipSetDevice(ctx->device));
  if (p.nBr * p.nchunk * (p.sum_j ? p.nj : 1) == 0) {
    WBX_HIP(hipMemsetAsync(out, 0, (size_t)nout * sizeof(double), ctx->stream));
    return 0;
  }
  WBX_REQUIRE(partial != nullptr && W != nullptr, "partial/W is NULL");
  if (p.sum_j || p.nj < 64) {
    const int fixed_j = p.sum_j ? 0 : 1;
    const int64_t grid = p.nA * p.nBk * p.nlane * (fixed_j ? p.nj : 1);
    WBX_REQUIRE(grid < (int64_t)1 << 31, "stage-2 grid too large");
    const int64_t ncontr = p.nBr * p.nchunk * (fixed_j ? 1 : p.nj);
    const int threads = ncontr >= 256 ? 256 : (ncontr >= 128 ? 128 : 64);
    int nsplit = 1;
    double* dst = out;
    const int64_t nrc = p.nBr * p.nchunk;
    if (!fixed_j && p.nj >= 64 && grid < 1024 && nrc * p.nj >= ((int64_t)1 << 16)) {
      int64_t want = (2048 + grid - 1) / grid;
      if (want > nrc) want = nrc;
      nsplit = (int)want;
      const size_t need = (size_t)grid * nsplit * p.nbin * sizeof(double);
      if (ctx->s2_scratch_size < need) {
        if (ctx->s2_scratch) {
          WBX_HIP(hipStreamSynchronize(ctx->stream));
          WBX_HIP(hipFree(ctx->s2_scratch));
          ctx->s2_scratch = nullptr;
          ctx->s2_scratch_size = 0;
        }
        WBX_HIP(hipMalloc(&ctx->s2_scratch, need));
        ctx->s2_scratch_size = need;
      }
      dst = reinterpret_cast<double*>(ctx->s2_scratch);
    }
    hipLaunchKernelGGL(wbx::s2_reduce_kernel, dim3((unsigned)(grid * nsplit)), dim3(threads), 0, ctx->stream, p, fixed_j,
                       nsplit, partial, W, dst);
    if (nsplit > 1) {
      WBX_HIP(hipGetLastError());
      const int64_t n = grid * p.nbin;
      hipLaunchKernelGGL(wbx::s2_bits_finish_kernel, dim3((unsigned)((n + 255) / 256)), dim3(256), 0, ctx->stream, grid,
                         nsplit, (int)p.nbin, dst, out);
    }
  } else {
    const int threads = p.nj >= 256 ? 256 : (p.nj >= 128 ? 128 : 64);
    const int njtile = (int)((p.nj + threads - 1) / threads);
    const int64_t grid = p.nA * p.nBk * p.nlane * njtile;
    WBX_REQUIRE(grid < (int64_t)1 << 31, "stage-2 grid too large");
    hipLaunchKernelGGL(wbx::s2_keepj_kernel, dim3((unsigned)grid), dim3(threads), 0, ctx->stream, p, njtile, partial,
                       W, out);
  }
  WBX_HIP(hipGetLastError());
  return 0;
}
```

weatherbenchx_amd/engine.py:

```python
from __future__ import annotations

import collections
import contextlib
import ctypes as C
import dataclasses
import os
from typing import Sequence

import numpy as np

from weatherbenchx_amd import _hip
from weatherbenchx_amd import planner
from weatherbenchx_amd import replay
from weatherbenchx_amd import xarray_lite as xr

_is_torch = xr._is_torch


class _Dev:

  def __init__(self, ptr, layout, dtype_code, keep, nbytes, fence=None):
    self.ptr, self.layout, self.dtype_code, self.keep, self.nbytes = ptr, layout, dtype_code, keep, nbytes
    self.fence = fence
    self.frozen = []
# ... 239 lines not shown
      store.clear()
    factors = None if w_da is None else w_da.__dict__.get('_wbx_factors')
    nbin = int(np.prod([w_da.sizes[d] for d in bin_dims], dtype=np.int64)) if (w_da is not None and bin_dims) else 1
    if factors is not None and BITS_MIN_BINS <= nbin <= 64:
      wt, bits, shape4, bin_shape = pack_bits(plan, factors[0], factors[1], bin_dims)
      store[sig] = _WOnDevice('bits', (ctx.upload(wt), ctx.upload(bits)), shape4, bin_shape)
      if SEPARABLE_BINNED_WEIGHTS and wt.shape[2] > 1 and np.array_equal(wt, np.broadcast_to(wt[:, :1, :], wt.shape)):
        store[sig].factored = (_hip.BINNED_WT_X_ONLY, ctx.upload(np.ascontiguousarray(wt[:, 0, :])))
      elif SEPARABLE_BINNED_WEIGHTS and np.array_equal(wt, np.broadcast_to(wt[:, :, :1], wt.shape)):
        store[sig].factored = (_hip.BINNED_WT_ROW_ONLY, ctx.upload(np.ascontiguousarray(wt[:, :, 0])))
    else:
      w, bin_shape = dense_w(plan, w_da, bin_dims)
      store[sig] = _WOnDevice('dense', (ctx.upload(w),), w.shape, bin_shape)
  return store[sig]


def _planned(ctx, kind, dims, sizes, layouts, reduce_dims, wdep, gather, flags, x_weights=None, one_wave=False, force_x=None):
  hit = _planned_inner(ctx, kind, dims, sizes, layouts, reduce_dims, wdep, gather, flags, x_weights, one_wave, force_x)
  rec = replay.active()
  if rec is not None and gather is not None:
    rec.note_gather(hit[1], lambda g: _planned_inner(ctx, kind, dims, sizes, layouts, reduce_dims, wdep, g, flags, x_weights,
                                                     one_wave, force_x)[1])
  return hit


def _planned_inner(ctx, kind, dims, sizes, layouts, reduce_dims, wdep, gather, flags, x_weights=None, one_wave=False, force_x=None):
  gsig = gbytes = None
  if gather is not None:
    gtable = np.ascontiguousarray(gather.table, dtype=np.int64)
    gsig = (tuple(gather.dims), gtable.shape, not bool(np.any(gtable % 4)))
    gbytes = gtable.tobytes()
    if not SWAP_GATHER_TABLES:
      gsig += (gbytes,)
  sig = (id(ctx), kind, bool(one_wave), force_x, tuple(dims), tuple(sizes[d] for d in dims),
         None if x_weights is None else hash(x_weights.tobytes()),
         tuple(None if l is None else (tuple(sorted(l.strides.items(), key=str)), l.itemsize, l.base_alignment % 16 == 0)
               for l in layouts),
         tuple(sorted(reduce_dims, key=str)), tuple(sorted(wdep, key=str)), flags, gsig)
  hit = _fast_plan_cache.get(sig)
  if hit is None:
    plan = planner.build_s1_plan(dims, sizes, layouts, reduce_dims, wdep_dims=wdep, gather=gather, flags=flags,
                                 allow_vec4=(kind in ('det', 'cont') and x_weights is None and force_x is None), force_x_dim=force_x,
                                 fold_x=False if x_weights is None else
                                 (True if kind == 'det' else ('point64' if one_wave else 'point')))
    if kind == 'cont' and plan.plane_rows > 0:
      plan = planner.build_s1_plan(dims, sizes, layouts, reduce_dims, wdep_dims=wdep, gather=gather, flags=flags,
                                   allow_vec4=False, force_x_dim=force_x)
    if x_weights is not None and plan.plane_rows > 0:
      assert not plan.x_kept and plan.vec == 1 and plan.nx == x_weights.size
      plan.x_weights = np.ascontiguousarray(x_weights, dtype=np.float64)
    if len(_fast_plan_cache) > 64:
      _fast_plan_cache.clear()
    hit = (plan, _device_plan(ctx, plan), {'built': gbytes})
    _fast_plan_cache[sig] = hit
  plan, dplan, variants = hit
  if gather is None or gbytes == variants['built']:
    return plan, dplan
  var = variants.get(gbytes)
  if var is None:
    gtab = planner.gather_table(plan.key_dims, plan.depth_dims, gather)
    if len(variants) > GATHER_VARIANTS_MAX:
      retired = {k: v for k, v in variants.items() if k not in ('built', 'retired')}
      built = variants['built']
      variants.clear()
      variants['built'], variants['retired'] = built, retired
    plan_v = dataclasses.replace(plan, gather_tab=gtab)
    rec = replay.active()
    if rec is not None:
      rec.paused += 1
    try:
      var = variants[gbytes] = (plan_v, _swap_gather_table(ctx, dplan, plan_v))
    finally:
      if rec is not None:
        rec.paused -= 1
  return var


def _swap_gather_table(ctx, dplan: _PlanOnDevice, plan_v: planner.S1Plan) -> _PlanOnDevice:
  return dplan.with_gather_table(ctx, plan_v.gather_tab)


SWAP_GATHER_TABLES = True
GATHER_VARIANTS_MAX = 512
_fast_plan_cache: dict = {}
_thr_cache: dict = {}
_count_cache: dict = {}
_const_roots: dict = {}


def register_constant(arr: np.ndarray) -> np.ndarray:
  arr.flags.writeable = False
  _const_roots[id(arr)] = arr
  return arr


def _constant_view_key(a):
  if not isinstance(a, np.ndarray) or a.flags.writeable:
    return None
  root = a
  while isinstance(root, np.ndarray) and root.base is not None:
    root = root.base
  if not isinstance(root, np.ndarray) or _const_roots.get(id(root)) is not root:
    return None
  return (id(root), a.__array_interface__['data'][0], a.shape, a.strides)
_scratch_bufs: dict = {}


def _scratch(ctx, slot: str, nbytes: int):
  key = (id(ctx), slot)
  buf = _scratch_bufs.get(key)
  if buf is None or buf.nbytes < nbytes:
    buf = ctx.alloc(int(nbytes * 1.25) + 256)
    _scratch_bufs[key] = buf
  return buf


def _threshold_table(ctx, thresholds):
  tkey = (ctx.device_id, np.asarray(thresholds, np.float64).tobytes())
  thr = _thr_cache.get(tkey)
  if thr is None:
    if len(_thr_cache) > 64:
      _thr_cache.clear()
    thr = _thr_cache[tkey] = ctx.upload(np.asarray(thresholds, np.float64))
  return thr


def contingency_available(ctx) -> bool:
  if not isinstance(ctx, _hip.Context):
    return False
  try:
    return getattr(ctx.lib, 'wbx_contingency_partial', None) is not None
  except AttributeError:
    return False


def ens_rps_available(ctx) -> bool:
  if not isinstance(ctx, _hip.Context):
    return False
  try:
    return getattr(ctx.lib, 'wbx_ens_rps_partial', None) is not None
  except AttributeError:
    return False


def ens_energy_available(ctx) -> bool:
  if not isinstance(ctx, _hip.Context):
    return False
  try:
    return getattr(ctx.lib, 'wbx_ens_energy_partial', None) is not None
  except AttributeError:
    return False


def new_context() -> _hip.Context:
  return _hip.Context(_hip.default_context().device_id)


def stage_inputs(ctx, arrays: Sequence[xr.DataArray]):
  arrays = [a for a in arrays if a is not None]
  dtype_code = _common_dtype([a.data for a in arrays])
  for a in arrays:
    if not (_is_torch(a.data) and a.data.is_cuda):
      _to_device(ctx, a, dtype_code)


ALTERNATE_STREAMS = os.environ.get('WBX_ALTERNATE_STREAMS', '1') != '0'
ALTERNATE_CHUNKS = True
ENS_PIPE = os.environ.get('WBX_ENS_PIPE', '1') != '0'
_stream_ring: list = []


def _launch_context(kind: str = 'det'):
  d = _deferred
  base = _hip.default_context()
  if d is None or not ALTERNATE_STREAMS or kind == 'det':
    return base
  if not _stream_ring or _stream_ring[0] is not base:
    _stream_ring[:] = [base, new_context()]
  if _accum is not None:
    return _stream_ring[_accum.launch_turn(len(_stream_ring))]
  d.turn = (d.turn + 1) % len(_stream_ring)
  return _stream_ring[d.turn]


def launch_contexts():
  base = _hip.default_context()
  return [base] + [c for c in _stream_ring if c is not base]


def known_contexts():
  return list(_hip.ALL_CONTEXTS or ())


def clear_caches():
  replay.invalidate_all()
  _stream_ring.clear()
  _plan_cache.clear()
  _w_cache.clear()
  _fast_plan_cache.clear()
  _count_cache.clear()
  _const_roots.clear()
  _scratch_bufs.clear()
  _thr_cache.clear()


_fusion_requests: dict = {}
_fusion_parks: list = []
FUSE_DET_SPECTRA = True
FUSE_DET_SPECTRA_LATFAST = os.environ.get('WBX_FUSE_DET_SPECTRA_LATFAST', '0') == '1'


def request_det_spectra(p_da, t_da, entry, ngroup: int):
  if FUSE_DET_SPECTRA:
    _fusion_requests[id(p_da)] = {'p': p_da, 't': t_da, 'entry': entry, 'ngroup': int(ngroup)}


def clear_det_spectra_requests():
  _fusion_requests.clear()
  for da in _fusion_parks:
    da.__dict__.pop('_wbx_fused_spectrum', None)
  _fusion_parks.clear()


def _fused_rows(plan: planner.S1Plan, entry):
  row_dims, row_shape = entry['row_dims'], entry['row_shape']
  key_dims = plan.key_dims
  if plan.ndepth != 1 or set(key_dims) | set(plan.depth_dims) != set(row_dims):
    return None
  idx = np.zeros((), dtype=np.int64)
  strides = {}
  mult = 1
  for d, n in zip(reversed(row_dims), reversed(row_shape)):
    strides[d] = mult
    mult *= n
  for d in key_dims:
    idx = idx[..., None] + np.arange(plan.sizes[d], dtype=np.int64) * strides[d]
  return np.ascontiguousarray(np.asarray(idx).reshape(-1))


def _fused_slab_rows(plan: planner.S1Plan, entry, nin: int):
  ckey = ('slabs', tuple(plan.key_dims), tuple(plan.sizes[d] for d in plan.key_dims), tuple(plan.xstride[:nin]))
  hit = entry['dev'].get(ckey)
  if hit is None:
    hit = False
    rows = _fused_rows(plan, entry)
    if rows is not None and rows.size == plan.nkey and plan.key_dims and plan.nchunk == 1 and not plan.x_kept:
      rps = int(plan.sizes[plan.key_dims[-1]])
      ok = rps >= 1 and all(plan.xstride[i] >= rps for i in range(nin))
      for i in range(nin):
        ko = plan.key_off[i]
        ok = ok and ko is not None and (rps == 1 or bool(np.all(np.diff(np.asarray(ko).reshape(-1, rps), axis=1) == 1)))
      if ok and plan.gather_key is not None and rps > 1:
        ok = bool(np.all(np.diff(np.asarray(plan.gather_key).reshape(-1, rps), axis=1) == 0))
      if ok:
        hit = rps
    entry['dev'][ckey] = hit
  return hit or None


def _fusion_latfast_plan(ctx, inputs, dims, sizes, layouts, reduce_dims, wdep, gather, func, dtype_code):
  if not FUSE_DET_SPECTRA_LATFAST:
    return None
  req = _fusion_requests.get(id(inputs[0]))
  if req is None or req['p'] is not inputs[0] or req['t'] is not inputs[1] or layouts[0] is None:
    return None
  lon = [d for d in dims if d not in req['entry']['row_dims']]
  if len(lon) != 1 or func not in (_hip.DET3, _hip.DET6) or dtype_code != _hip.F32 or ctx is not _hip.default_context():
    return None
  lon = lon[0]
  if (sizes[lon] != 1440 or lon not in set(reduce_dims) or lon in wdep or layouts[0].stride(lon) == 1
      or (gather is not None and lon in gather.dims)):
    return None
  nin = _hip.DET_INPUTS[func]
  if any(layouts[i] is None for i in range(nin)):
    return None
  plan, dplan = _planned(ctx, 'det', dims, sizes, layouts, reduce_dims, wdep, gather, 0, force_x=lon)
  if plan.ndepth != 1 or _fused_slab_rows(plan, req['entry'], nin) is None:
    return None
  return plan, dplan


class _FoldedS2:

  def __init__(self, res):
    self.res = res


FOLD_DET_SPECTRA = True


def _try_det_spectra(ctx, inputs, dplan, plan, devs, dtype_code, func, make_out, fold=None):
  if not _fusion_requests or inputs is None:
    return False
  req = _fusion_requests.get(id(inputs[0]))
  if req is None or req['p'] is not inputs[0] or req['t'] is not inputs[1]:
    return False
  nin = _hip.DET_INPUTS[func]
  if (func not in (_hip.DET3, _hip.DET6) or dtype_code != _hip.F32 or plan.nx != 1440 or plan.x_kept or plan.ndepth != 1
      or plan.nchunk != 1 or plan.flags or plan.x_weights is not None or plan.x_dim is None or ctx is not _hip.default_context()):
    return False
  entry, ngroup = req['entry'], req['ngroup']
  rps = None
  if any(plan.xstride[i] != 1 for i in range(nin)):
    rps = _fused_slab_rows(plan, entry, nin)
    if rps is None:
      return False
  fkey = ('fused', tuple(plan.key_dims), tuple(plan.sizes[d] for d in plan.key_dims))
  bufs = entry['dev'].get(fkey)
  if bufs is None:
    rows = _fused_rows(plan, entry)
    if rows is None or rows.size != plan.nkey:
      entry['dev'][fkey] = bufs = False
    else:
      g = np.ascontiguousarray(np.asarray(entry['group'])[rows], dtype=np.int32)
      sc = np.ascontiguousarray(np.asarray(entry['scale'])[rows], dtype=np.float64)
      entry['dev'][fkey] = bufs = (ctx.upload(g), ctx.upload(sc), g)
  if bufs is False:
    return False
  folded = None
  if FOLD_DET_SPECTRA and fold is not None and rps is None:
    s2, w_da, bin_dims, w_buf = fold
    nl = _hip.DET_LANES[func]
    if (s2.nBk == 1 and s2.nbin == 1 and s2.nj == 1 and not plan.x_kept and s2.nchunk == 1 and s2.nlane == nl and s2.nA == ngroup
        and s2.nA * s2.nBr == plan.nkey and w_buf.kind == 'dense'):
      key2 = fkey + ('fold', id(w_buf))
      folded = entry['dev'].get(key2)
      if folded is None:
        folded = False
        w, _ = dense_w(plan, w_da, bin_dims)
        if w.shape == (1, s2.nBr, 1, 1) and np.array_equal(bufs[2], np.repeat(np.arange(s2.nA, dtype=np.int32), s2.nBr)):
          folded = (ctx.upload(np.ascontiguousarray(np.tile(w[0, :, 0, 0], s2.nA))), w_buf)
        entry['dev'][key2] = folded
      folded = folded or None
  del _fusion_requests[id(inputs[0])]
  replay.keep(bufs[:2], folded[0] if folded else None, dplan, devs[2] if nin > 2 else None)
  nk = 721
  pw_p = ctx.alloc(max(ngroup * nk, 1) * 8)
  pw_t = ctx.alloc(max(ngroup * nk, 1) * 8)
  ptr = lambda d: C.c_void_p(d.ptr) if d is not None else None

  det_out = out = None
  if folded:
    det_shape = fold[0].out_shape()
    det_out = _scratch(ctx, 's2out', int(np.prod(det_shape, dtype=np.int64)) * 8)
  else:
    out = make_out()

  def call():
    if folded:
      _hip.check(ctx.lib.wbx_det_spectrum_folded(ctx.handle, C.byref(dplan.struct), func, dtype_code, ptr(devs[0]), ptr(devs[1]),
                                                 ptr(devs[2]) if nin > 2 else None, C.c_void_p(bufs[0].ptr), C.c_void_p(bufs[1].ptr),
                                                 C.c_void_p(folded[0].ptr), int(ngroup), C.c_void_p(det_out.ptr),
                                                 C.c_void_p(pw_p.ptr), C.c_void_p(pw_t.ptr)), 'wbx_det_spectrum_folded')
    elif rps is None:
      _hip.check(ctx.lib.wbx_det_spectrum(ctx.handle, C.byref(dplan.struct), func, dtype_code, ptr(devs[0]), ptr(devs[1]),
                                          ptr(devs[2]) if nin > 2 else None, C.c_void_p(bufs[0].ptr), C.c_void_p(bufs[1].ptr),
                                          int(ngroup), C.c_void_p(out.ptr), C.c_void_p(pw_p.ptr), C.c_void_p(pw_t.ptr)),
                 'wbx_det_spectrum')
    else:
      _hip.check(ctx.lib.wbx_det_spectrum_slabs(ctx.handle, C.byref(dplan.struct), func, dtype_code, ptr(devs[0]), ptr(devs[1]),
                                                ptr(devs[2]) if nin > 2 else None, int(rps), C.c_void_p(bufs[0].ptr),
                                                C.c_void_p(bufs[1].ptr), int(ngroup), C.c_void_p(out.ptr), C.c_void_p(pw_p.ptr),
                                                C.c_void_p(pw_t.ptr)), 'wbx_det_spectrum_slabs')
  timed_launch(ctx, call, kind='det_spectrum', rows=int(plan.nkey), func=int(func), slab_rows=int(rps or 0), folded=bool(folded))
  for da, buf in ((req['p'], pw_p), (req['t'], pw_t)):
    da.__dict__['_wbx_fused_spectrum'] = {'ctx': ctx, 'ptr': buf.ptr, 'buf': buf, 'ngroup': ngroup, 'cache': entry['dev']}
    _fusion_parks.append(da)
  return _FoldedS2((det_out.ptr, det_shape)) if folded else out


EnsArgs = collections.namedtuple('EnsArgs', 'm mstride algo')
RpsEnsArgs = collections.namedtuple('RpsEnsArgs', 'm mstride')
Ens2Args = collections.namedtuple('Ens2Args', 'm mstride n_t tstride')
CatArgs = collections.namedtuple('CatArgs', 'func ncat m mstride thr cstride')
ContArgs = collections.namedtuple('ContArgs', 'nthr thr')
RpsArgs = collections.namedtuple('RpsArgs', 'nthr p_thr t_thr right')
EnergyArgs = collections.namedtuple('EnergyArgs', 'm mstride norm_len p_norm_stride t_norm_stride')
_table_ptr = lambda buf: C.c_void_p(buf.ptr) if buf is not None else None


def _cat_operands(ctx, devs, func, ens, cat, mdim):
  field = cat.get('thr_field') is not None
  thr = _threshold_table(ctx, cat['thresholds']) if cat.get('thresholds') is not None and not field else None
  return int(cat['ncat']), None, CatArgs(cat['func'], int(cat['ncat']), cat.get('M', 1) if mdim else 1,
                                         devs[0].layout.stride(mdim) if mdim else 0, thr,
                                         devs[2].layout.stride(cat['cat_dim']) if field else None)


def _cont_operands(ctx, devs, func, ens, cat, mdim):
  nthr = int(np.asarray(cat['thresholds']).size)
  if not 1 <= nthr <= _hip.CONT_MAX_THRESHOLDS:
    raise ValueError(f'one contingency launch takes 1..{_hip.CONT_MAX_THRESHOLDS} thresholds (got {nthr})')
  return _hip.CONT_CELLS * nthr, None, ContArgs(nthr, _threshold_table(ctx, cat['thresholds']))


def _erps_operands(ctx, devs, func, ens, cat, mdim):
  nthr = int(np.asarray(cat['p_thresholds']).size)
  if not 1 <= nthr <= _hip.ERPS_MAX_THRESHOLDS or int(np.asarray(cat['t_thresholds']).size) != nthr:
    raise ValueError(f'one ensemble RPS launch takes 1..{_hip.ERPS_MAX_THRESHOLDS} prediction and as many target thresholds '
                     f"(got {nthr} and {int(np.asarray(cat['t_thresholds']).size)})")
  if not 1 <= int(ens['M']) <= _hip.ERPS_MAX_MEMBERS:
    raise ValueError(f"one ensemble RPS launch takes 1..{_hip.ERPS_MAX_MEMBERS} members (got {ens['M']})")
  return 1, RpsEnsArgs(ens['M'], devs[0].layout.stride(mdim)), RpsArgs(
      nthr, _threshold_table(ctx, cat['p_thresholds']), _threshold_table(ctx, cat['t_thresholds']), bool(cat['right_inclusive']))


def norm_run(layout, dims, sizes):
  live = sorted(((abs(layout.stride(d)), layout.stride(d), int(sizes[d])) for d in dims if int(sizes[d]) != 1), key=lambda v: v[0])
  length = int(np.prod([int(sizes[d]) for d in dims], dtype=np.int64))
  if not live:
    return length, 0
  if live[0][1] <= 0:
    return None
  for (_, s0, n0), (_, s1, _) in zip(live, live[1:]):
    if s1 != s0 * n0:
      return None
  return length, live[0][1]


def _enrg_operands(ctx, devs, func, ens, cat, mdim):
  if not 2 <= int(ens['M']) <= _hip.ENRG_MAX_MEMBERS:
    raise ValueError(f"one energy score launch takes 2..{_hip.ENRG_MAX_MEMBERS} members (got {ens['M']})")
  runs = [norm_run(devs[i].layout, ens['norm_dims'], ens['norm_sizes']) for i in (0, 1)]
  if runs[0] is None or runs[1] is None:
    raise ValueError(f"the norm dims {ens['norm_dims']} are not one strided run of the inputs as they are stored")
  return _hip.ENRG_LANES, EnergyArgs(ens['M'], devs[0].layout.stride(mdim), runs[0][0], runs[0][1], runs[1][1]), None


_Kind = collections.namedtuple('_Kind', 'operands keep call')
_KINDS = {
    'det': _Kind(lambda ctx, devs, func, ens, cat, mdim: (_hip.DET_LANES[func], None, None), (),
                 lambda d, out, dt, func, ens, cat: ('wbx_det_partial', (func, dt, d[0], d[1], d[2], d[3], out))),
    'ens': _Kind(lambda ctx, devs, func, ens, cat, mdim:
                 (_hip.ENS_LANES, EnsArgs(ens['M'], devs[0].layout.stride(mdim), ens['algo']), None), (),
                 lambda d, out, dt, func, ens, cat: ('wbx_ens_partial', (dt, *map(int, ens), d[0], d[1], d[3], out))),
    'ens2': _Kind(lambda ctx, devs, func, ens, cat, mdim:
                  (_hip.ENS2_LANES, Ens2Args(ens['M'], devs[0].layout.stride(mdim), ens['N'], devs[1].layout.stride(mdim)), None), (),
                  lambda d, out, dt, func, ens, cat: ('wbx_ens2_partial', (dt, *map(int, ens), d[0], d[1], d[3], out))),
    'cat': _Kind(_cat_operands, ('thr',),
                 lambda d, out, dt, func, ens, cat:
                 ('wbx_cat_exceed_field', (dt, int(cat.ncat), int(cat.m), int(cat.mstride), d[0], d[1], d[2], int(cat.cstride), d[3], out))
                 if cat.cstride is not None else
                 ('wbx_cat_partial', (int(cat.func), dt, int(cat.ncat), int(cat.m), int(cat.mstride), d[0], d[1], _table_ptr(cat.thr),
                                      d[3], out))),
    'cont': _Kind(_cont_operands, ('thr',),
                  lambda d, out, dt, func, ens, cat:
                  ('wbx_contingency_partial', (dt, int(cat.nthr), d[0], d[1], _table_ptr(cat.thr), d[3], out))),
    'erps': _Kind(_erps_operands, ('p_thr', 't_thr'),
                  lambda d, out, dt, func, ens, cat:
                  ('wbx_ens_rps_partial', (dt, *map(int, ens), int(cat.nthr), _table_ptr(cat.p_thr), _table_ptr(cat.t_thr),
                                           int(bool(cat.right)), d[0], d[1], d[3], out))),
    'enrg': _Kind(_enrg_operands, (),
                  lambda d, out, dt, func, ens, cat: ('wbx_ens_energy_partial', (dt, *map(int, ens), d[0], d[1], d[3], out))),
}


def _run_s1(ctx, kind: str, dplan: _PlanOnDevice, plan: planner.S1Plan, devs: Sequence[_Dev | None], dtype_code: int,
            nlanes_total: int, func: int = 0, ens=None, cat=None, inputs=None, fold=None):
  n = int(np.prod(plan.partial_shape(nlanes_total), dtype=np.int64))
  if kind == 'det' and _fusion_requests:
    hit = _try_det_spectra(ctx, inputs, dplan, plan, devs, dtype_code, func, lambda: _scratch(ctx, 'partial', n * 8), fold)
    if hit is not False:
      return hit
  out = _scratch(ctx, 'partial', n * 8)

  def call():
    name, args = _KINDS[kind].call([_table_ptr(d) for d in devs], C.c_void_p(out.ptr), dtype_code, func, ens, cat)
    _hip.check(getattr(ctx.lib, name)(ctx.handle, C.byref(dplan.struct), *args), name)
  if S1_EVENT_LOG is None:
    call()
  else:
    timed_launch(ctx, call, kind=kind, vec=plan.vec, x_kept=plan.x_kept, plane_rows=plan.plane_rows,
                 x_weighted=plan.x_weights is not None, flat=plan.x_weights is not None and plan.plane_rows > 0,
                 grid=plan.nkey * plan.nchunk, block=plan.block_threads, algo=int(EnsArgs(*ens).algo) if kind == 'ens' else None,
                 flags=int(plan.flags))
  return out


S1_EVENT_LOG = None
S1_EVENT_REPEAT = 1
S1_EVENT_MARKS = False


def timed_launch(ctx, call, **entry):
  if S1_EVENT_LOG is None:
    call()
  elif S1_EVENT_MARKS:
    i0 = ctx.mark()
    call()
    S1_EVENT_LOG.append(dict(entry, ms=None, reps=1, marks=(ctx, i0, ctx.mark())))
  else:
    reps = max(1, int(S1_EVENT_REPEAT))
    ctx.timer_start()
    for _ in range(reps):
      call()
    S1_EVENT_LOG.append(dict(entry, ms=ctx.timer_stop() / reps, reps=reps))


def resolve_event_marks(log):
  ctxs = {}
  for e in log:
    if e.get('marks') is not None:
      ctx, i0, i1 = e.pop('marks')
      e['ms'] = ctx.mark_elapsed(i0, i1)
      ctxs[id(ctx)] = ctx
  for ctx in ctxs.values():
    ctx.marks_reset()
  return log


def _run_map(ctx, kind: str, dplan, plan: planner.S1Plan, devs, dtype_code: int, lane: int, func: int = 0,
             ens=None) -> np.ndarray:
  n = plan.nkey * plan.ndepth * plan.nx
  out = ctx.alloc(n * 8)
  ptr = lambda d: C.c_void_p(d.ptr) if d is not None else None
  if kind == 'det':
    _hip.check(ctx.lib.wbx_det_map(ctx.handle, C.byref(dplan.struct), func, dtype_code, lane, ptr(devs[0]),
                                   ptr(devs[1]), ptr(devs[2]), C.c_void_p(out.ptr)), 'wbx_det_map')
  else:
    m, mstride, algo = ens
    _hip.check(ctx.lib.wbx_ens_map(ctx.handle, C.byref(dplan.struct), dtype_code, int(m), int(mstride), int(algo),
                                   lane, ptr(devs[0]), ptr(devs[1]), C.c_void_p(out.ptr)), 'wbx_ens_map')
  return ctx.download(out.ptr, (n,), np.float64)


class DeferredResults:

  def __init__(self):
    self.ctxs = {}
    self.turn = 0
    self.keepalive = []

  def mark(self):
    fences = [ctx.fence() for ctx in self.ctxs.values()]
    keep, self.ctxs, self.keepalive = self.keepalive, {}, []
    return ResultFence(fences, keep)


class ResultFence:

  def __init__(self, fences=(), keepalive=()):
    self._fences = list(fences)
    self._keepalive = list(keepalive)

  def wait(self):
    for f in self._fences:
      f.wait()
    self._fences = []
    self._keepalive = []

  def __del__(self):
    try:
      self.wait()
    except Exception:
      pass


_deferred: DeferredResults | None = None


@contextlib.contextmanager
def deferred_results():
  global _deferred
  prev, mine = _deferred, DeferredResults()
  _deferred = mine
  try:
    yield mine
  finally:
    _deferred = prev
    mine.mark().wait()


def deferred_active() -> DeferredResults | None:
  return _deferred


@contextlib.contextmanager
def synchronous_results():
  global _deferred, _accum
  saved, _deferred = _deferred, None
  saved_acc, _accum = _accum, None
  try:
    yield
  finally:
    _deferred, _accum = saved, saved_acc


class _HostResult:

  def __init__(self, view):
    self.view = view


class _AccumulatedInPlace:

  def __init__(self, ptr):
    self.ptr = ptr


FUSED_ACC_ADD = True


def _result_target(ctx, shape, scratch_name, can_accumulate=False):
  n = int(np.prod(shape, dtype=np.int64))
  if can_accumulate:
    if FUSED_ACC_ADD and _accum is not None and n and S1_EVENT_LOG is None:
      ptr = _accum.slot_pointer(ctx, n)
      if ptr is not None:
        return ptr, _AccumulatedInPlace(ptr), True
    return _result_target(ctx, shape, scratch_name) + (False,)
  if _deferred is not None and _accum is None and n:
    view = ctx.pinned_result(shape)
    return view.ctypes.data, _HostResult(view)
  out = _scratch(ctx, scratch_name, n * 8)
  return out.ptr, out.ptr


# ... 579 lines not shown
```

Baseline: 120.5 billion.

## Fold ensemble stage-2 contraction into stage-1 kernel via last-block reduction

```diff
diff --git a/include/wbx.h b/include/wbx.h
--- a/include/wbx.h
+++ b/include/wbx.h
@@ -135,6 +135,11 @@
 int wbx_contract_bits(wbx_ctx* ctx, const wbx_s2_plan* plan, const double* partial, const double* wt,
                       const uint64_t* bits, double* out);
 
+#define WBX_NOT_FOLDED 1
+int wbx_ens_partial_folded(wbx_ctx* ctx, const wbx_s1_plan* plan, int dtype, int M, int64_t member_stride,
+                           int algo , const void* p, const void* t, double* partial_out,
+                           const wbx_s2_plan* s2plan, const double* W, double* out, int add);
+
 typedef enum wbx_cat_func { WBX_CAT_EXCEED = 0, WBX_CAT_RANK = 1 } wbx_cat_func;
 int wbx_cat_partial(wbx_ctx* ctx, const wbx_s1_plan* plan, int func, int dtype, int ncat, int M,
                     int64_t member_stride, const void* p, const void* t, const double* thresholds,
@@ -215,7 +220,7 @@
   WBX_FN_CONTRACT = 6, WBX_FN_CONTRACT_BITS = 7, WBX_FN_DET_BINNED = 8, WBX_FN_ENS_BINNED = 9, WBX_FN_ZONAL_SPECTRUM = 10,
   WBX_FN_ZONAL_SPECTRUM_SLABS = 11, WBX_FN_DET_SPECTRUM = 12, WBX_FN_DET_SPECTRUM_SLABS = 13, WBX_FN_ACC_ADD = 14,
   WBX_FN_MEMSET = 15, WBX_FN_MEMCPY_D2D = 16, WBX_FN_CTX_WAIT_FENCE = 17, WBX_FN_FENCE_RECORD = 18, WBX_FN_DET_SPECTRUM_FOLDED = 19,
-  WBX_FN_CONTINGENCY_PARTIAL = 20, WBX_FN_ENS_RPS_PARTIAL = 21, WBX_FN_ENS_ENERGY_PARTIAL = 22
+  WBX_FN_CONTINGENCY_PARTIAL = 20, WBX_FN_ENS_RPS_PARTIAL = 21, WBX_FN_ENS_ENERGY_PARTIAL = 22, WBX_FN_ENS_PARTIAL_FOLDED = 23
 } wbx_fn;
 #define WBX_CALL_MAX_ARGS 20
 typedef struct wbx_call {
diff --git a/weatherbenchx_amd/_hip.py b/weatherbenchx_amd/_hip.py
--- a/weatherbenchx_amd/_hip.py
+++ b/weatherbenchx_amd/_hip.py
@@ -29,6 +29,8 @@
 FLAG_MASKED, FLAG_SKIPNA, FLAG_FAIR, FLAG_SKIPNA_ENS = 1, 2, 4, 8
 BINNED_W_ON_X, BINNED_WT_X_ONLY, BINNED_WT_ROW_ONLY, BINNED_MASK_ON_W, BINNED_TWIN_MASK = 1, 2, 4, 8, 16
 BINNED_ACCUMULATE = 32
+NOT_FOLDED = 1
+ENS_FOLD_MAX_BINS = 8
 
 EXPORTED_SYMBOLS = (
     'wbx_abi_version', 'wbx_last_error', 'wbx_device_count', 'wbx_ctx_create', 'wbx_ctx_destroy',
@@ -41,14 +43,15 @@
     'wbx_comm_unique_id', 'wbx_comm_create', 'wbx_comm_destroy', 'wbx_comm_info', 'wbx_acc_allreduce', 'wbx_acc_read',
     'wbx_acc_reset', 'wbx_det_spectrum', 'wbx_det_spectrum_slabs', 'wbx_ens_binned', 'wbx_ens_binned_atoms_size', 'wbx_ens_binned_atoms',
     'wbx_ens2_partial', 'wbx_cat_exceed_field', 'wbx_chunk_replay', 'wbx_host_transpose', 'wbx_clock_probe', 'wbx_det_spectrum_folded',
-    'wbx_contingency_partial', 'wbx_ens_rps_partial', 'wbx_ens_energy_partial',
+    'wbx_contingency_partial', 'wbx_ens_rps_partial', 'wbx_ens_energy_partial', 'wbx_ens_partial_folded',
 )
 
 FN_IDS = {'wbx_det_partial': 1, 'wbx_ens_partial': 2, 'wbx_ens2_partial': 3, 'wbx_cat_partial': 4, 'wbx_cat_exceed_field': 5,
           'wbx_contract': 6, 'wbx_contract_bits': 7, 'wbx_det_binned': 8, 'wbx_ens_binned': 9, 'wbx_zonal_spectrum': 10,
           'wbx_zonal_spectrum_slabs': 11, 'wbx_det_spectrum': 12, 'wbx_det_spectrum_slabs': 13, 'wbx_acc_add': 14,
           'wbx_memset': 15, 'wbx_memcpy_d2d': 16, 'wbx_ctx_wait_fence': 17, 'wbx_fence_record': 18, 'wbx_det_spectrum_folded': 19,
-          'wbx_contingency_partial': 20, 'wbx_ens_rps_partial': 21, 'wbx_ens_energy_partial': 22}
+          'wbx_contingency_partial': 20, 'wbx_ens_rps_partial': 21, 'wbx_ens_energy_partial': 22, 'wbx_ens_partial_folded': 23}
+OPTIONAL_SYMBOLS = frozenset({'wbx_ens_partial_folded'})
 CALL_MAX_ARGS = 20
 QUERY_FNS = frozenset({'wbx_s1_partial_len', 'wbx_binned_atoms_size', 'wbx_ens_binned_atoms_size', 'wbx_last_error',
                        'wbx_abi_version', 'wbx_device_count', 'wbx_comm_info'})
@@ -180,6 +183,7 @@
         'wbx_s1_partial_len': [C.POINTER(S1PlanStruct), i32, C.POINTER(i64)],
         'wbx_det_partial': [vp, C.POINTER(S1PlanStruct), i32, i32, vp, vp, vp, vp, vp],
         'wbx_ens_partial': [vp, C.POINTER(S1PlanStruct), i32, i32, i64, i32, vp, vp, vp, vp],
+        'wbx_ens_partial_folded': [vp, C.POINTER(S1PlanStruct), i32, i32, i64, i32, vp, vp, vp, C.POINTER(S2PlanStruct), vp, vp, i32],
         'wbx_contract': [vp, C.POINTER(S2PlanStruct), vp, vp, vp],
         'wbx_contract_bits': [vp, C.POINTER(S2PlanStruct), vp, vp, vp, vp],
         'wbx_det_binned': [vp, C.POINTER(S1PlanStruct), i32, i32, vp, vp, vp, vp, vp, vp, i64, i64, i64, C.c_int32, C.c_int32, vp, vp],
@@ -205,8 +209,14 @@
     protos['wbx_chunk_replay'] = [vp, i32, vp, i32, vp, i32]
     protos['wbx_host_transpose'] = [vp, vp, i64, i64, i64, C.c_int32]
     protos['wbx_clock_probe'] = [vp, C.c_int32, C.POINTER(C.c_double)]
-    for name, argtypes in protos.items():
-      fn = getattr(lib, name)
+    for name, argtypes in list(protos.items()):
+      try:
+        fn = getattr(lib, name)
+      except AttributeError:
+        if name not in OPTIONAL_SYMBOLS:
+          raise
+        del protos[name]
+        continue
       fn.argtypes = argtypes
       fn.restype = i32
     PROTOS.update(protos)
diff --git a/weatherbenchx_amd/csrc/wbx_common.hpp b/weatherbenchx_amd/csrc/wbx_common.hpp
--- a/weatherbenchx_amd/csrc/wbx_common.hpp
+++ b/weatherbenchx_amd/csrc/wbx_common.hpp
@@ -23,6 +23,8 @@
   void* atoms_clean = nullptr;
   void* patch_counters = nullptr;
   size_t patch_counters_size = 0;
+  void* fold_counters = nullptr;
+  size_t fold_counters_size = 0;
   hipEvent_t* marks = nullptr;
   int marks_used = 0, marks_made = 0, marks_cap = 0;
 };
@@ -99,9 +101,28 @@
   return __hiloint2double(__builtin_amdgcn_readlane(__double2hiint(t), 63), __builtin_amdgcn_readlane(__double2loint(t), 63));
 }
 
+template <typename T>
+__device__ __forceinline__ void st_dev(T* p, T v) {
+  __hip_atomic_store(p, v, __ATOMIC_RELAXED, __HIP_MEMORY_SCOPE_AGENT);
+}
+template <typename T>
+__device__ __forceinline__ T ld_dev(const T* p) {
+  return __hip_atomic_load(p, __ATOMIC_RELAXED, __HIP_MEMORY_SCOPE_AGENT);
 }
 
-#define WBX_HIP(expr)                                                                   \
+__device__ __forceinline__ double ld_sc1(__amdgpu_buffer_rsrc_t rs, uint32_t byte_offset) {
+  typedef unsigned int u2 __attribute__((ext_vector_type(2)));
+  const u2 v = __builtin_amdgcn_raw_buffer_load_b64(rs, (int)byte_offset, 0, 1 << 4);
+  return __hiloint2double((int)v.y, (int)v.x);
+}
+
+__device__ __forceinline__ double s2_madd(double acc, double v, double w) { return __builtin_fma(v, w, acc); }
+
+inline int s2_reduce_threads(int64_t ncontr) { return ncontr >= 256 ? 256 : (ncontr >= 128 ? 128 : 64); }
+
+}
+
+#define WBX_HIP(expr)                                                                  \
   do {                                                                                  \
     hipError_t _e = (expr);                                                             \
     if (_e != hipSuccess)                                                               \
diff --git a/weatherbenchx_amd/csrc/wbx_ctx.hip b/weatherbenchx_amd/csrc/wbx_ctx.hip
--- a/weatherbenchx_amd/csrc/wbx_ctx.hip
+++ b/weatherbenchx_amd/csrc/wbx_ctx.hip
@@ -71,6 +71,7 @@
   if (ctx->s2_scratch) (void)hipFree(ctx->s2_scratch);
   if (ctx->aidm_scratch) (void)hipFree(ctx->aidm_scratch);
   if (ctx->patch_counters) (void)hipFree(ctx->patch_counters);
+  if (ctx->fold_counters) (void)hipFree(ctx->fold_counters);
   delete static_cast<std::set<const void*>*>(ctx->atoms_clean);
   if (ctx->ev_start) (void)hipEventDestroy(ctx->ev_start);
   if (ctx->ev_stop) (void)hipEventDestroy(ctx->ev_stop);
diff --git a/weatherbenchx_amd/csrc/wbx_ens.hip b/weatherbenchx_amd/csrc/wbx_ens.hip
--- a/weatherbenchx_amd/csrc/wbx_ens.hip
+++ b/weatherbenchx_amd/csrc/wbx_ens.hip
@@ -4,7 +4,8 @@
 namespace wbx {
 
 static int ens_common(wbx_ctx* ctx, const wbx_s1_plan* plan, int dtype, int M, int64_t member_stride, int algo,
-                      const void* p, const void* t, const uint8_t* mask, double* out, bool map, int lane) {
+                      const void* p, const void* t, const uint8_t* mask, double* out, bool map, int lane,
+                      const EnsFoldArgs* fold = nullptr) {
   if (int rc = s1_begin("", ctx, plan)) return rc;
   WBX_REQUIRE(plan->vec == 1, "ensemble kernels use vec=1");
   WBX_REQUIRE(M >= 1, "ensemble size must be >= 1 (got %d)", M);
@@ -16,20 +17,22 @@
   a.M = M;
   a.mstride = member_stride;
   a.lane = lane;
-  if (dtype == WBX_F64) return launch_ens_op<EnsOpGeneric<double>>(ctx, plan, a, map);
+  if (dtype == WBX_F64) return fold ? WBX_NOT_FOLDED : launch_ens_op<EnsOpGeneric<double>>(ctx, plan, a, map);
   WBX_REQUIRE(dtype == WBX_F32, "unknown dtype %d", dtype);
+  if (fold && M > 64) return WBX_NOT_FOLDED;
   if (plan->flags & WBX_FLAG_SKIPNA_ENS) {
     static const bool generic = getenv("WBX_ENS_SKIPNA_GENERIC") && atoi(getenv("WBX_ENS_SKIPNA_GENERIC")) != 0;
+    if (fold && generic) return WBX_NOT_FOLDED;
     if (generic || M > 64) return launch_ens_op<EnsOpGeneric<float>>(ctx, plan, a, map);
     algo = WBX_ENS_SKIPNA_SORT;
   }
-  if (M == 51) return launch_ens_m51(ctx, plan, a, algo, map);
-  if (M == 50) return launch_ens_m50(ctx, plan, a, algo, map);
-  if (M <= 4) return launch_ens_m4(ctx, plan, a, algo, map);
-  if (M <= 8) return launch_ens_m8(ctx, plan, a, algo, map);
-  if (M <= 16) return launch_ens_m16(ctx, plan, a, algo, map);
-  if (M <= 32) return launch_ens_m32(ctx, plan, a, algo, map);
-  if (M <= 64) return launch_ens_m64(ctx, plan, a, algo, map);
+  if (M == 51) return launch_ens_m51(ctx, plan, a, algo, map, fold);
+  if (M == 50) return launch_ens_m50(ctx, plan, a, algo, map, fold);
+  if (M <= 4) return launch_ens_m4(ctx, plan, a, algo, map, fold);
+  if (M <= 8) return launch_ens_m8(ctx, plan, a, algo, map, fold);
+  if (M <= 16) return launch_ens_m16(ctx, plan, a, algo, map, fold);
+  if (M <= 32) return launch_ens_m32(ctx, plan, a, algo, map, fold);
+  if (M <= 64) return launch_ens_m64(ctx, plan, a, algo, map, fold);
   return launch_ens_op<EnsOpGeneric<float>>(ctx, plan, a, map);
 }
 
@@ -38,6 +41,28 @@
 extern "C" int wbx_ens_partial(wbx_ctx* ctx, const wbx_s1_plan* plan, int dtype, int M, int64_t member_stride,
                                int algo, const void* p, const void* t, const uint8_t* mask, double* partial_out) {
   return wbx::ens_common(ctx, plan, dtype, M, member_stride, algo, p, t, mask, partial_out, false, 0);
+}
+
+extern "C" int wbx_ens_partial_folded(wbx_ctx* ctx, const wbx_s1_plan* plan, int dtype, int M, int64_t member_stride, int algo,
+                                      const void* p, const void* t, double* partial_out, const wbx_s2_plan* s2plan, const double* W,
+                                      double* out, int add) {
+  using namespace wbx;
+  WBX_REQUIRE(ctx != nullptr && plan != nullptr && s2plan != nullptr, "wbx_ens_partial_folded: ctx / plan / s2plan is NULL");
+  const wbx_s2_plan& s = *s2plan;
+  if (plan->x_kept || (plan->flags & (WBX_FLAG_MASKED | WBX_FLAG_SKIPNA)) || s.nj != 1 || s.nbin < 1 || s.nbin > ENS_FOLD_MAX_BINS || s.nlane != WBX_ENS_LANES || s.nA < 1 || s.nBk < 1 || s.nBr < 1 ||
+      s.nchunk != plan->nchunk || s.nA * s.nBk * s.nBr != plan->nkey || plan->nkey * plan->nchunk >= (int64_t)1 << 31 ||
+      plan->ndepth <= 0 || plan->nx <= 0 || s.nBr * s.nchunk * WBX_ENS_LANES * 8 >= (int64_t)1 << 31)
+    return WBX_NOT_FOLDED;
+  WBX_REQUIRE(W != nullptr && out != nullptr, "wbx_ens_partial_folded: W / out is NULL");
+  EnsFoldArgs f = {};
+  f.W = W;
+  f.out = out;
+  f.nBr = (int32_t)s.nBr;
+  f.nBk = (int32_t)s.nBk;
+  f.nbin = (int32_t)s.nbin;
+  f.threads = s2_reduce_threads(s.nBr * s.nchunk);
+  f.add = add != 0;
+  return ens_common(ctx, plan, dtype, M, member_stride, algo, p, t, nullptr, partial_out, false, 0, &f);
 }
 
 extern "C" int wbx_ens_map(wbx_ctx* ctx, const wbx_s1_plan* plan, int dtype, int M, int64_t member_stride, int algo,
diff --git a/weatherbenchx_amd/csrc/wbx_ens_atoms.hpp b/weatherbenchx_amd/csrc/wbx_ens_atoms.hpp
--- a/weatherbenchx_amd/csrc/wbx_ens_atoms.hpp
+++ b/weatherbenchx_amd/csrc/wbx_ens_atoms.hpp
@@ -17,25 +17,10 @@
 constexpr int ENS_ATOMS_G1 = 4;
 constexpr int ENS_ATOMS_G2 = 16;
 
-template <typename T>
-__device__ __forceinline__ void st_dev(T* p, T v) {
-  __hip_atomic_store(p, v, __ATOMIC_RELAXED, __HIP_MEMORY_SCOPE_AGENT);
-}
-template <typename T>
-__device__ __forceinline__ T ld_dev(const T* p) {
-  return __hip_atomic_load(p, __ATOMIC_RELAXED, __HIP_MEMORY_SCOPE_AGENT);
-}
-
 __device__ __forceinline__ void wave_lds_order() {
   __builtin_amdgcn_fence(__ATOMIC_RELEASE, "wavefront");
   __builtin_amdgcn_wave_barrier();
   __builtin_amdgcn_fence(__ATOMIC_ACQUIRE, "wavefront");
-}
-
-__device__ __forceinline__ double ld_sc1(__amdgpu_buffer_rsrc_t rs, uint32_t byte_offset) {
-  typedef unsigned int u2 __attribute__((ext_vector_type(2)));
-  const u2 v = __builtin_amdgcn_raw_buffer_load_b64(rs, (int)byte_offset, 0, 1 << 4);
-  return __hiloint2double((int)v.y, (int)v.x);
 }
 
 struct EnsAtomsArgs {
diff --git a/weatherbenchx_amd/csrc/wbx_ens_impl.hpp b/weatherbenchx_amd/csrc/wbx_ens_impl.hpp
--- a/weatherbenchx_amd/csrc/wbx_ens_impl.hpp
+++ b/weatherbenchx_amd/csrc/wbx_ens_impl.hpp
@@ -1,5 +1,6 @@
 #pragma once
 #include <cmath>
+#include <cstddef>
 #include <cstdlib>
 
 #include "wbx_s1.hpp"
@@ -447,9 +448,111 @@
 constexpr int ENS_PIPE_NLDS = 50;
 constexpr int ENS_PIPE_WAVES = 3;
 constexpr int ENS_PIPE_SKIPNA_WAVES = 3;
+
+struct EnsFoldArgs {
+  const double* W;
+  double* out;
+  uint32_t* counters;
+  int32_t nBr, nBk, nbin;
+  int32_t threads;
+  int32_t add;
+  int32_t nsub;
+};
+constexpr int ENS_FOLD_SUB = 16, ENS_FOLD_PAD = 32;
+inline int ens_fold_nsub(int64_t ncontr) { return ncontr > ENS_FOLD_SUB ? (int)((ncontr + ENS_FOLD_SUB - 1) / ENS_FOLD_SUB) : 0; }
+inline size_t ens_fold_counter_words(int64_t ngroup, int nsub) {
+  return nsub ? (size_t)ngroup * (size_t)(nsub + 1) * ENS_FOLD_PAD : (size_t)ngroup;
+}
+struct EnsPipeArgSegment {
+  S1Args a;
+  int R;
+  EnsFoldArgs f;
+};
+constexpr int ENS_FOLD_MAX_BINS = 8;
+
+template <int NL>
+__device__ __forceinline__ void ens_fold_finish(const S1Args& a, const EnsFoldArgs& f, int64_t key, int chunk, int lane) {
+  constexpr int NSET = 4, U = 2;
+  const uint32_t group = (uint32_t)key / (uint32_t)f.nBr;
+  const uint32_t nchunk = (uint32_t)a.nchunk;
+  const uint32_t ncontr = (uint32_t)f.nBr * nchunk;
+  auto last_of = [&](uint32_t* counter, uint32_t total) -> bool {
+    asm volatile("s_waitcnt vmcnt(0)" ::: "memory");
+    uint32_t seen = 0;
+    if (lane == 0) seen = __hip_atomic_fetch_add(counter, 1u, __ATOMIC_RELAXED, __HIP_MEMORY_SCOPE_AGENT);
+    seen = (uint32_t)__builtin_amdgcn_readfirstlane((int)seen);
+    if (seen != total - 1) return false;
+    if (lane == 0) st_dev(counter, 0u);
+    return true;
+  };
+  if (f.nsub) {
+    uint32_t* const base = f.counters + (size_t)group * (size_t)(f.nsub + 1) * ENS_FOLD_PAD;
+    const uint32_t c = ((uint32_t)key - group * (uint32_t)f.nBr) * nchunk + (uint32_t)chunk;
+    const uint32_t sub = c / ENS_FOLD_SUB, left = ncontr - sub * ENS_FOLD_SUB;
+    if (!last_of(base + (size_t)(1 + sub) * ENS_FOLD_PAD, left < ENS_FOLD_SUB ? left : (uint32_t)ENS_FOLD_SUB)) return;
+    if (!last_of(base, (uint32_t)f.nsub)) return;
+  } else if (!last_of(f.counters + group, ncontr)) {
+    return;
+  }
+
+  const uint32_t T = (uint32_t)f.threads;
+  const int nset = (int)(T >> 6);
+  const double* wbase = f.W + (int64_t)(group % (uint32_t)f.nBk) * f.nBr * f.nbin;
+  const __amdgpu_buffer_rsrc_t rs = __builtin_amdgcn_make_buffer_rsrc(a.out + (int64_t)group * ncontr * NL, 0, 0x7fffffff, 0x00020000);
+  const uint32_t nround = (ncontr + T - 1) / T;
+#pragma unroll 1
+  for (int g = 0; g < f.nbin; ++g) {
+    double acc[NSET][NL];
+#pragma unroll
+    for (int k = 0; k < NSET; ++k)
+#pragma unroll
+      for (int l = 0; l < NL; ++l) acc[k][l] = 0.0;
+#pragma unroll 1
+    for (uint32_t j0 = 0; j0 < nround; j0 += U) {
+      double v[U][NSET][NL], w[U][NSET];
+      bool on[U][NSET];
+#pragma unroll
+      for (int u = 0; u < U; ++u)
+#pragma unroll
+        for (int k = 0; k < NSET; ++k) {
+          const uint32_t c = (j0 + u) * T + (uint32_t)k * 64u + (uint32_t)lane;
+          on[u][k] = k < nset && j0 + u < nround && c < ncontr;
+          const uint32_t cc = on[u][k] ? c : 0u;
+#pragma unroll
+          for (int l = 0; l < NL; ++l) v[u][k][l] = ld_sc1(rs, (cc * NL + l) * 8u);
+          w[u][k] = wbase[(int64_t)(cc / nchunk) * f.nbin + g];
+        }
+#pragma unroll
+      for (int u = 0; u < U; ++u)
+#pragma unroll
+        for (int k = 0; k < NSET; ++k)
+#pragma unroll
+          for (int l = 0; l < NL; ++l) acc[k][l] = on[u][k] ? s2_madd(acc[k][l], v[u][k][l], w[u][k]) : acc[k][l];
+    }
+    double mine = 0.0;
+#pragma unroll
+    for (int l = 0; l < NL; ++l) {
+      double s = 0.0;
+#pragma unroll
+      for (int k = 0; k < NSET; ++k) {
+        const double ws = wave_sum(acc[k][l]);
+        s = k < nset ? s + ws : s;
+      }
+      if (lane == l) mine = s;
+    }
+    if (lane < NL) {
+      double* q = f.out + ((int64_t)group * NL + lane) * f.nbin + g;
+      *q = f.add ? *q + mine : mine;
+    }
+  }
+}
+
 template <int MP, bool EXACT, int ALGO, bool FLAT>
 __global__ void __launch_bounds__(64, ALGO == WBX_ENS_SKIPNA_SORT ? ENS_PIPE_SKIPNA_WAVES : ENS_PIPE_WAVES)
-ens_pipe_kernel(S1Args a, int R) {
+ens_pipe_kernel(S1Args a, int R, EnsFoldArgs fold_block) {
+  const uint64_t kargs = (uint64_t)__builtin_amdgcn_kernarg_segment_ptr();
+  uint32_t kargs_lo = (uint32_t)kargs, kargs_hi = (uint32_t)(kargs >> 32);
+  asm volatile("" : "+v"(kargs_lo), "+v"(kargs_hi));
   using Op = EnsOpF32<MP, EXACT, ALGO>;
   constexpr int NA = Op::NACC;
   constexpr int NLDS = MP < ENS_PIPE_NLDS ? MP : ENS_PIPE_NLDS;
@@ -566,11 +669,23 @@
       for (int l = 0; l < NA; ++l) acc[l] += valid ? val[l] : 0.0;
     }
   }
+  asm volatile("" : "+v"(kargs_lo), "+v"(kargs_hi));
+  const uint64_t kargs2 = ((uint64_t)(uint32_t)__builtin_amdgcn_readfirstlane((int)kargs_hi) << 32) |
+                          (uint32_t)__builtin_amdgcn_readfirstlane((int)kargs_lo);
+  const const_ptr<EnsFoldArgs> fp = (const_ptr<EnsFoldArgs>)(kargs2 + offsetof(EnsPipeArgSegment, f));
+  EnsFoldArgs f;
+  f.W = fp->W, f.out = fp->out, f.counters = fp->counters;
+  f.nBr = fp->nBr, f.nBk = fp->nBk, f.nbin = fp->nbin, f.threads = fp->threads, f.add = fp->add, f.nsub = fp->nsub;
 #pragma unroll
   for (int l = 0; l < NA; ++l) {
     const double v = wave_sum(acc[l]);
-    if (lane == l) a.out[(key * a.nchunk + chunk) * NA + l] = v;
-  }
+    if (lane == l) {
+      double* q = a.out + (key * a.nchunk + chunk) * NA + l;
+      if (f.counters) st_dev(q, v);
+      else *q = v;
+    }
+  }
+  if (f.counters) ens_fold_finish<NA>(a, f, key, chunk, lane);
 }
 
 #pragma clang diagnostic pop
@@ -596,12 +711,35 @@
   return (double)plan->nx * (double)plan->plane_rows * 4.0 < 4294967296.0;
 }
 
+inline int ens_fold_counters(wbx_ctx* ctx, size_t n, uint32_t** out) {
+  if (ctx->fold_counters_size < n) {
+    if (ctx->fold_counters) {
+      WBX_HIP(hipStreamSynchronize(ctx->stream));
+      WBX_HIP(hipFree(ctx->fold_counters));
+      ctx->fold_counters = nullptr;
+      ctx->fold_counters_size = 0;
+    }
+    const size_t cap = n < 4096 ? 4096 : n * 2;
+    WBX_HIP(hipMalloc(&ctx->fold_counters, cap * sizeof(uint32_t)));
+    WBX_HIP(hipMemsetAsync(ctx->fold_counters, 0, cap * sizeof(uint32_t), ctx->stream));
+    ctx->fold_counters_size = cap;
+  }
+  *out = reinterpret_cast<uint32_t*>(ctx->fold_counters);
+  return 0;
+}
+
 template <int MP, bool EXACT, int ALGO, bool FLAT = false>
-int launch_ens_pipe(wbx_ctx* ctx, const wbx_s1_plan* plan, S1Args& a) {
+int launch_ens_pipe(wbx_ctx* ctx, const wbx_s1_plan* plan, S1Args& a, const EnsFoldArgs* fold) {
   const int64_t grid = plan->nkey * plan->nchunk;
   WBX_REQUIRE(grid < (int64_t)1 << 31, "grid too large (%lld blocks)", (long long)grid);
+  EnsFoldArgs f = {};
+  if (fold) {
+    f = *fold;
+    f.nsub = ens_fold_nsub((int64_t)f.nBr * plan->nchunk);
+    if (int rc = ens_fold_counters(ctx, ens_fold_counter_words(plan->nkey / f.nBr, f.nsub), &f.counters)) return rc;
+  }
   hipLaunchKernelGGL((ens_pipe_kernel<MP, EXACT, ALGO, FLAT>), dim3((unsigned)grid), dim3(64), 0, ctx->stream, a,
-                     FLAT ? plan->plane_rows : 0);
+                     FLAT ? plan->plane_rows : 0, f);
   WBX_HIP(hipGetLastError());
   return 0;
 }
@@ -621,9 +759,11 @@
 }
 
 template <int MP, bool EXACT>
-int launch_ens_bucket(wbx_ctx* ctx, const wbx_s1_plan* plan, S1Args& a, int algo, bool map) {
-  if (!map && algo == WBX_ENS_SORT && ens_pipe_ok(plan, a)) return launch_ens_pipe<MP, EXACT, WBX_ENS_SORT>(ctx, plan, a);
-  if (!map && algo == WBX_ENS_SORT && ens_pipe_flat_ok(plan, a)) return launch_ens_pipe<MP, EXACT, WBX_ENS_SORT, true>(ctx, plan, a);
+int launch_ens_bucket(wbx_ctx* ctx, const wbx_s1_plan* plan, S1Args& a, int algo, bool map, const EnsFoldArgs* fold) {
+  if (!map && algo == WBX_ENS_SORT && ens_pipe_ok(plan, a)) return launch_ens_pipe<MP, EXACT, WBX_ENS_SORT>(ctx, plan, a, fold);
+  if (!map && algo == WBX_ENS_SORT && ens_pipe_flat_ok(plan, a)) return launch_ens_pipe<MP, EXACT, WBX_ENS_SORT, true>(ctx, plan, a, fold);
+  if (!map && algo == WBX_ENS_SKIPNA_SORT && ens_pipe_ok(plan, a, true)) return launch_ens_pipe<MP, EXACT, WBX_ENS_SKIPNA_SORT>(ctx, plan, a, fold);
+  if (fold) return WBX_NOT_FOLDED;
   if (algo == WBX_ENS_SORT) return launch_ens_op<EnsOpF32<MP, EXACT, WBX_ENS_SORT>>(ctx, plan, a, map);
   if (algo == WBX_ENS_DIAG_LOADONLY) {
     if (!EXACT || map) return fail(WBX_ERR_INVALID, "the load-only diagnostic exists for the exact-M partial kernels only");
@@ -638,17 +778,16 @@
       return fail(WBX_ERR_INVALID, "the LDS-tiled pair-form diagnostic exists for M = 51 only");
     }
   }
-  if (!map && algo == WBX_ENS_SKIPNA_SORT && ens_pipe_ok(plan, a, true)) return launch_ens_pipe<MP, EXACT, WBX_ENS_SKIPNA_SORT>(ctx, plan, a);
   if (algo == WBX_ENS_SKIPNA_SORT) return launch_ens_op<EnsOpF32<MP, EXACT, WBX_ENS_SKIPNA_SORT>>(ctx, plan, a, map);
   return launch_ens_op<EnsOpF32<MP, EXACT, WBX_ENS_PAIRWISE>>(ctx, plan, a, map);
 }
 
-int launch_ens_m4(wbx_ctx*, const wbx_s1_plan*, S1Args&, int, bool);
-int launch_ens_m8(wbx_ctx*, const wbx_s1_plan*, S1Args&, int, bool);
-int launch_ens_m16(wbx_ctx*, const wbx_s1_plan*, S1Args&, int, bool);
-int launch_ens_m32(wbx_ctx*, const wbx_s1_plan*, S1Args&, int, bool);
-int launch_ens_m64(wbx_ctx*, const wbx_s1_plan*, S1Args&, int, bool);
-int launch_ens_m50(wbx_ctx*, const wbx_s1_plan*, S1Args&, int, bool);
-int launch_ens_m51(wbx_ctx*, const wbx_s1_plan*, S1Args&, int, bool);
-
-}
+int launch_ens_m4(wbx_ctx*, const wbx_s1_plan*, S1Args&, int, bool, const EnsFoldArgs*);
+int launch_ens_m8(wbx_ctx*, const wbx_s1_plan*, S1Args&, int, bool, const EnsFoldArgs*);
+int launch_ens_m16(wbx_ctx*, const wbx_s1_plan*, S1Args&, int, bool, const EnsFoldArgs*);
+int launch_ens_m32(wbx_ctx*, const wbx_s1_plan*, S1Args&, int, bool, const EnsFoldArgs*);
+int launch_ens_m64(wbx_ctx*, const wbx_s1_plan*, S1Args&, int, bool, const EnsFoldArgs*);
+int launch_ens_m50(wbx_ctx*, const wbx_s1_plan*, S1Args&, int, bool, const EnsFoldArgs*);
+int launch_ens_m51(wbx_ctx*, const wbx_s1_plan*, S1Args&, int, bool, const EnsFoldArgs*);
+
+}
diff --git a/weatherbenchx_amd/csrc/wbx_ens_m16.hip b/weatherbenchx_amd/csrc/wbx_ens_m16.hip
--- a/weatherbenchx_amd/csrc/wbx_ens_m16.hip
+++ b/weatherbenchx_amd/csrc/wbx_ens_m16.hip
@@ -1,8 +1,8 @@
 #include "wbx_ens_atoms.hpp"
 #include "wbx_ens_impl.hpp"
 namespace wbx {
-int launch_ens_m16(wbx_ctx* ctx, const wbx_s1_plan* plan, S1Args& a, int algo, bool map) {
-  return launch_ens_bucket<16, false>(ctx, plan, a, algo, map);
+int launch_ens_m16(wbx_ctx* ctx, const wbx_s1_plan* plan, S1Args& a, int algo, bool map, const EnsFoldArgs* fold) {
+  return launch_ens_bucket<16, false>(ctx, plan, a, algo, map, fold);
 }
 int launch_ens_atoms_m16(wbx_ctx* ctx, const wbx_s1_plan* plan, S1Args& a, const EnsBinnedCall& c) {
   return launch_ens_atoms<16, false>(ctx, plan, a, c);
diff --git a/weatherbenchx_amd/csrc/wbx_ens_m32.hip b/weatherbenchx_amd/csrc/wbx_ens_m32.hip
--- a/weatherbenchx_amd/csrc/wbx_ens_m32.hip
+++ b/weatherbenchx_amd/csrc/wbx_ens_m32.hip
@@ -1,8 +1,8 @@
 #include "wbx_ens_atoms.hpp"
 #include "wbx_ens_impl.hpp"
 namespace wbx {
-int launch_ens_m32(wbx_ctx* ctx, const wbx_s1_plan* plan, S1Args& a, int algo, bool map) {
-  return launch_ens_bucket<32, false>(ctx, plan, a, algo, map);
+int launch_ens_m32(wbx_ctx* ctx, const wbx_s1_plan* plan, S1Args& a, int algo, bool map, const EnsFoldArgs* fold) {
+  return launch_ens_bucket<32, false>(ctx, plan, a, algo, map, fold);
 }
 int launch_ens_atoms_m32(wbx_ctx* ctx, const wbx_s1_plan* plan, S1Args& a, const EnsBinnedCall& c) {
   return launch_ens_atoms<32, false>(ctx, plan, a, c);
diff --git a/weatherbenchx_amd/csrc/wbx_ens_m4.hip b/weatherbenchx_amd/csrc/wbx_ens_m4.hip
--- a/weatherbenchx_amd/csrc/wbx_ens_m4.hip
+++ b/weatherbenchx_amd/csrc/wbx_ens_m4.hip
@@ -1,8 +1,8 @@
 #include "wbx_ens_atoms.hpp"
 #include "wbx_ens_impl.hpp"
 namespace wbx {
-int launch_ens_m4(wbx_ctx* ctx, const wbx_s1_plan* plan, S1Args& a, int algo, bool map) {
-  return launch_ens_bucket<4, false>(ctx, plan, a, algo, map);
+int launch_ens_m4(wbx_ctx* ctx, const wbx_s1_plan* plan, S1Args& a, int algo, bool map, const EnsFoldArgs* fold) {
+  return launch_ens_bucket<4, false>(ctx, plan, a, algo, map, fold);
 }
 int launch_ens_atoms_m4(wbx_ctx* ctx, const wbx_s1_plan* plan, S1Args& a, const EnsBinnedCall& c) {
   return launch_ens_atoms<4, false>(ctx, plan, a, c);
diff --git a/weatherbenchx_amd/csrc/wbx_ens_m50.hip b/weatherbenchx_amd/csrc/wbx_ens_m50.hip
--- a/weatherbenchx_amd/csrc/wbx_ens_m50.hip
+++ b/weatherbenchx_amd/csrc/wbx_ens_m50.hip
@@ -1,8 +1,8 @@
 #include "wbx_ens_atoms.hpp"
 #include "wbx_ens_impl.hpp"
 namespace wbx {
-int launch_ens_m50(wbx_ctx* ctx, const wbx_s1_plan* plan, S1Args& a, int algo, bool map) {
-  return launch_ens_bucket<50, true>(ctx, plan, a, algo, map);
+int launch_ens_m50(wbx_ctx* ctx, const wbx_s1_plan* plan, S1Args& a, int algo, bool map, const EnsFoldArgs* fold) {
+  return launch_ens_bucket<50, true>(ctx, plan, a, algo, map, fold);
 }
 int launch_ens_atoms_m50(wbx_ctx* ctx, const wbx_s1_plan* plan, S1Args& a, const EnsBinnedCall& c) {
   return launch_ens_atoms<50, true>(ctx, plan, a, c);
diff --git a/weatherbenchx_amd/csrc/wbx_ens_m51.hip b/weatherbenchx_amd/csrc/wbx_ens_m51.hip
--- a/weatherbenchx_amd/csrc/wbx_ens_m51.hip
+++ b/weatherbenchx_amd/csrc/wbx_ens_m51.hip
@@ -1,8 +1,8 @@
 #include "wbx_ens_atoms.hpp"
 #include "wbx_ens_impl.hpp"
 namespace wbx {
-int launch_ens_m51(wbx_ctx* ctx, const wbx_s1_plan* plan, S1Args& a, int algo, bool map) {
-  return launch_ens_bucket<51, true>(ctx, plan, a, algo, map);
+int launch_ens_m51(wbx_ctx* ctx, const wbx_s1_plan* plan, S1Args& a, int algo, bool map, const EnsFoldArgs* fold) {
+  return launch_ens_bucket<51, true>(ctx, plan, a, algo, map, fold);
 }
 int launch_ens_atoms_m51(wbx_ctx* ctx, const wbx_s1_plan* plan, S1Args& a, const EnsBinnedCall& c) {
   return launch_ens_atoms<51, true>(ctx, plan, a, c);
diff --git a/weatherbenchx_amd/csrc/wbx_ens_m64.hip b/weatherbenchx_amd/csrc/wbx_ens_m64.hip
--- a/weatherbenchx_amd/csrc/wbx_ens_m64.hip
+++ b/weatherbenchx_amd/csrc/wbx_ens_m64.hip
@@ -1,8 +1,8 @@
 #include "wbx_ens_atoms.hpp"
 #include "wbx_ens_impl.hpp"
 namespace wbx {
-int launch_ens_m64(wbx_ctx* ctx, const wbx_s1_plan* plan, S1Args& a, int algo, bool map) {
-  return launch_ens_bucket<64, false>(ctx, plan, a, algo, map);
+int launch_ens_m64(wbx_ctx* ctx, const wbx_s1_plan* plan, S1Args& a, int algo, bool map, const EnsFoldArgs* fold) {
+  return launch_ens_bucket<64, false>(ctx, plan, a, algo, map, fold);
 }
 int launch_ens_atoms_m64(wbx_ctx* ctx, const wbx_s1_plan* plan, S1Args& a, const EnsBinnedCall& c) {
   return launch_ens_atoms<64, false>(ctx, plan, a, c);
diff --git a/weatherbenchx_amd/csrc/wbx_ens_m8.hip b/weatherbenchx_amd/csrc/wbx_ens_m8.hip
--- a/weatherbenchx_amd/csrc/wbx_ens_m8.hip
+++ b/weatherbenchx_amd/csrc/wbx_ens_m8.hip
@@ -1,8 +1,8 @@
 #include "wbx_ens_atoms.hpp"
 #include "wbx_ens_impl.hpp"
 namespace wbx {
-int launch_ens_m8(wbx_ctx* ctx, const wbx_s1_plan* plan, S1Args& a, int algo, bool map) {
-  return launch_ens_bucket<8, false>(ctx, plan, a, algo, map);
+int launch_ens_m8(wbx_ctx* ctx, const wbx_s1_plan* plan, S1Args& a, int algo, bool map, const EnsFoldArgs* fold) {
+  return launch_ens_bucket<8, false>(ctx, plan, a, algo, map, fold);
 }
 int launch_ens_atoms_m8(wbx_ctx* ctx, const wbx_s1_plan* plan, S1Args& a, const EnsBinnedCall& c) {
   return launch_ens_atoms<8, false>(ctx, plan, a, c);
diff --git a/weatherbenchx_amd/csrc/wbx_replay.hip b/weatherbenchx_amd/csrc/wbx_replay.hip
--- a/weatherbenchx_amd/csrc/wbx_replay.hip
+++ b/weatherbenchx_amd/csrc/wbx_replay.hip
@@ -51,6 +51,7 @@
     switch (c.fn) {
       WBX_REPLAY_CASE(WBX_FN_DET_PARTIAL, wbx_det_partial)
       WBX_REPLAY_CASE(WBX_FN_ENS_PARTIAL, wbx_ens_partial)
+      WBX_REPLAY_CASE(WBX_FN_ENS_PARTIAL_FOLDED, wbx_ens_partial_folded)
       WBX_REPLAY_CASE(WBX_FN_ENS2_PARTIAL, wbx_ens2_partial)
       WBX_REPLAY_CASE(WBX_FN_CAT_PARTIAL, wbx_cat_partial)
       WBX_REPLAY_CASE(WBX_FN_CAT_EXCEED_FIELD, wbx_cat_exceed_field)
diff --git a/weatherbenchx_amd/csrc/wbx_s2.hip b/weatherbenchx_amd/csrc/wbx_s2.hip
--- a/weatherbenchx_amd/csrc/wbx_s2.hip
+++ b/weatherbenchx_amd/csrc/wbx_s2.hip
@@ -59,7 +59,7 @@
         const double* w = wbase + (br * p.nj + j) * p.nbin + b0;
 #pragma unroll
         for (int g = 0; g < BG; ++g)
-          if (b0 + g < p.nbin) acc[g] += v * w[g];
+          if (b0 + g < p.nbin) acc[g] = s2_madd(acc[g], v, w[g]);
       }
     }
 #pragma unroll
@@ -272,7 +272,7 @@
     const int64_t grid = p.nA * p.nBk * p.nlane * (fixed_j ? p.nj : 1);
     WBX_REQUIRE(grid < (int64_t)1 << 31, "stage-2 grid too large");
     const int64_t ncontr = p.nBr * p.nchunk * (fixed_j ? 1 : p.nj);
-    const int threads = ncontr >= 256 ? 256 : (ncontr >= 128 ? 128 : 64);
+    const int threads = wbx::s2_reduce_threads(ncontr);
     int nsplit = 1;
     double* dst = out;
     const int64_t nrc = p.nBr * p.nchunk;
diff --git a/weatherbenchx_amd/engine.py b/weatherbenchx_amd/engine.py
--- a/weatherbenchx_amd/engine.py
+++ b/weatherbenchx_amd/engine.py
@@ -415,6 +415,15 @@
     return False
 
 
+def ens_fold_available(ctx) -> bool:
+  if not isinstance(ctx, _hip.Context):
+    return False
+  try:
+    return getattr(ctx.lib, 'wbx_ens_partial_folded', None) is not None
+  except AttributeError:
+    return False
+
+
 def new_context() -> _hip.Context:
   return _hip.Context(_hip.default_context().device_id)
 
@@ -550,6 +559,52 @@
 
 
 FOLD_DET_SPECTRA = True
+FOLD_ENS_S2 = True
+
+
+def _ens_fold_ok(ctx, plan: planner.S1Plan, dtype_code: int, nlanes_total: int, ens, fold) -> bool:
+  if not FOLD_ENS_S2 or not ENS_PIPE or not ens_fold_available(ctx):
+    return False
+  s2, _, _, w_buf = fold
+  m, _, algo = EnsArgs(*ens)
+  if (w_buf.kind != 'dense' or s2.nj != 1 or not 1 <= s2.nbin <= _hip.ENS_FOLD_MAX_BINS or s2.nlane != _hip.ENS_LANES
+      or nlanes_total != _hip.ENS_LANES or dtype_code != _hip.F32 or not 1 <= int(m) <= 64 or s2.nA * s2.nBk * s2.nBr != plan.nkey
+      or plan.nkey < 1 or s2.nchunk != plan.nchunk or plan.nkey * plan.nchunk >= 1 << 31):
+    return False
+  skipna_ens = bool(plan.flags & _hip.FLAG_SKIPNA_ENS)
+  if (plan.x_kept or plan.block_threads != 64 or plan.ndepth <= 0 or plan.nx <= 0 or plan.flags & (_hip.FLAG_MASKED | _hip.FLAG_SKIPNA)
+      or (int(algo) != _hip.ENS_SORT and not skipna_ens)):
+    return False
+  if plan.x_weights is None:
+    return plan.xstride[0] >= 0 and plan.xstride[1] >= 0 and plan.nx * plan.xstride[0] * 4 < 1 << 32
+  return (not skipna_ens and plan.plane_rows > 0 and plan.nx <= 2048 and plan.ndepth % plan.plane_rows == 0
+          and plan.xstride[0] == 1 and plan.xstride[1] == 1 and plan.nx * plan.plane_rows * 4 < 1 << 32)
+
+
+def _run_ens_folded(ctx, dplan, plan: planner.S1Plan, devs, dtype_code: int, ens, fold, partial):
+  s2 = fold[0]
+  st = _hip.S2PlanStruct(s2.nA, s2.nBk, s2.nBr, s2.nchunk, s2.nlane, s2.nj, s2.nbin, int(s2.sum_j))
+  shape = s2.out_shape()
+  out_ptr, handle, add = _result_target(ctx, shape, 's2out', can_accumulate=True)
+  m, mstride, algo = EnsArgs(*ens)
+  status = []
+
+  def call():
+    rc = ctx.lib.wbx_ens_partial_folded(ctx.handle, C.byref(dplan.struct), dtype_code, int(m), int(mstride), int(algo),
+                                        _table_ptr(devs[0]), _table_ptr(devs[1]), C.c_void_p(partial.ptr), C.byref(st),
+                                        C.c_void_p(fold[3].bufs[0].ptr), C.c_void_p(out_ptr), int(bool(add)))
+    if rc != _hip.NOT_FOLDED:
+      _hip.check(rc, 'wbx_ens_partial_folded')
+    status.append(rc)
+  timed_launch(ctx, call, kind='ens', vec=plan.vec, x_kept=plan.x_kept, plane_rows=plan.plane_rows,
+               x_weighted=plan.x_weights is not None, flat=plan.x_weights is not None and plan.plane_rows > 0,
+               grid=plan.nkey * plan.nchunk, block=plan.block_threads, algo=int(algo), flags=int(plan.flags), folded=True)
+  if status[-1] == _hip.NOT_FOLDED:
+    rec = _hip.RECORDER
+    if rec is not None:
+      rec.refuse('wbx_ens_partial_folded did not fold (a record replays every call it saw)')
+    return None
+  return _FoldedS2((handle, shape))
 
 
 def _try_det_spectra(ctx, inputs, dplan, plan, devs, dtype_code, func, make_out, fold=None):
@@ -726,6 +781,10 @@
     if hit is not False:
       return hit
   out = _scratch(ctx, 'partial', n * 8)
+  if kind == 'ens' and fold is not None and _ens_fold_ok(ctx, plan, dtype_code, nlanes_total, ens, fold):
+    hit = _run_ens_folded(ctx, dplan, plan, devs, dtype_code, ens, fold, out)
+    if hit is not None:
+      return hit
 
   def call():
     name, args = _KINDS[kind].call([_table_ptr(d) for d in devs], C.c_void_p(out.ptr), dtype_code, func, ens, cat)
```

New measurement: 120.0 billion. No clear change (-0.4%).
